# NVIDIA-AI-IOT/redtail

Hardware: AMD Instinct MI355X
Metric: stereo pairs/sec, ResNet18-2D 1257x369 (higher is better)
Workload: dtype f32

## Files before the change

include/rt_stereo.h:

```cpp
#ifndef RT_STEREO_H
#define RT_STEREO_H

#include <stddef.h>
#include <stdint.h>

#ifdef __cplusplus
extern "C" {
#endif

typedef void* rtStream;

enum { RT_F32 = 0, RT_F16 = 1 };
enum { RT_NCHW = 0, RT_NC2HW2 = 1 };
enum { RT_ACT_NONE = 0, RT_ACT_ELU = 1, RT_ACT_SIGMOID = 2 };
enum { RT_E_BADARG = -1, RT_E_UNSUPPORTED = -2, RT_E_NODEVICE = -3, RT_E_NOMEM = -4, RT_E_RUNTIME = -5 };

const char* rt_last_error_string(void);
const char* rt_backend_name(void);
int rt_device_count(void);
int rt_set_device(int ordinal);

int rt_malloc(void** dptr, size_t bytes);
int rt_free(void* dptr);
int rt_memcpy_h2d(void* dst, const void* src, size_t bytes, rtStream stream);
// ... 67 lines not shown
int rt_preprocess_frames_u8_lr(const void* left_u8, const void* right_u8, int src_h, int src_w, int64_t src_step, int encoding,
                               void* left_dst, void* right_dst, int dst_h, int dst_w, int batch, rtStream stream);
enum { RT_DISP_NET = 0, RT_DISP_PIXELS_F32 = 1, RT_DISP_KITTI_U16 = 2 };
int rt_lr_consistency(const void* net_disp, int batch, int H, int W, float scale, float max_diff_px, void* out, int out_kind,
                      void* mask_u8, void* right_out, void* valid_count, rtStream stream);

size_t rt_speckle_workspace_bytes(int batch, int H, int W);
int rt_disparity_speckle(const void* disp_px, const void* mask_u8, int batch, int H, int W, int max_size, float max_diff_px,
                         void* out, void* out_mask_u8, void* valid_count, void* workspace, size_t workspace_bytes, rtStream stream);

int rt_preprocess_frames_u8_cv(const void* left_u8, const void* right_u8, int src_h, int src_w, int64_t src_step, int encoding,
                               void* left_dst, void* right_dst, int dst_h, int dst_w, int batch, int mirror_twin, rtStream stream);
int rt_disparity_to_frame(const void* disp_px, const void* mask_u8, int batch, int H, int W, void* out, int out_kind, int out_h,
                          int out_w, void* out_mask_u8, void* valid_count, rtStream stream);

typedef struct rtStereoCamera {
    float fx, fy, cx, cy;
    float baseline;
    float doffs;
} rtStereoCamera;
enum { RT_DEPTH_M_F32 = 0, RT_DEPTH_MM_U16 = 1 };
size_t rt_points_workspace_bytes(int batch, int out_h, int out_w);
int rt_disparity_to_points(const void* disp_px, const void* mask_u8, int batch, int H, int W, int out_h, int out_w,
                           const rtStereoCamera* cam, float min_depth, float max_depth, const void* color_u8, int64_t color_step,
                           int encoding, void* disp_out, int disp_kind, void* out_mask_u8, void* valid_count, void* depth, int depth_kind,
                           void* points, void* points_compact, void* count, void* workspace, size_t workspace_bytes, rtStream stream);

typedef struct rtVoxelGrid { float origin[3]; float leaf[3]; int dims[3]; } rtVoxelGrid;
size_t rt_voxel_workspace_bytes(int batch, int capacity, const rtVoxelGrid* grid);
int rt_points_voxel_grid(const void* points, const void* count, int batch, int capacity, const rtVoxelGrid* grid, int min_points,
                         void* voxels, int out_capacity, void* out_count, void* out_cell_u32, void* out_n_u32,
                         void* workspace, size_t workspace_bytes, rtStream stream);

typedef struct rtRectifyCamera {
    double fx, fy, cx, cy;
    double d[8];
    double iR[9];
} rtRectifyCamera;
int rt_rectify_camera_from_info(const double K[9], const double* D, int n_d, const double R[9], const double P[12], rtRectifyCamera* out);
int rt_rectify_frames_u8(const void* left_u8, const void* right_u8, int src_h, int src_w, int64_t src_step, int encoding,
                         const rtRectifyCamera* cam_left, const rtRectifyCamera* cam_right,
                         void* left_dst, void* right_dst, int dst_h, int dst_w, int64_t dst_step, int batch, rtStream stream);
int rt_rectify_maps(const rtRectifyCamera* cam, int dst_h, int dst_w, void* map_x_f32, void* map_y_f32, rtStream stream);
int rt_remap_frames_u8(const void* left_u8, const void* right_u8, int src_h, int src_w, int64_t src_step, int encoding,
                       const void* map_x_left, const void* map_y_left, const void* map_x_right, const void* map_y_right,
                       void* left_dst, void* right_dst, int dst_h, int dst_w, int64_t dst_step, int batch, rtStream stream);

enum { RT_WIRE_MONO8 = 16, RT_WIRE_MONO16 = 17,
       RT_WIRE_BAYER_RGGB8 = 18, RT_WIRE_BAYER_BGGR8 = 19, RT_WIRE_BAYER_GBRG8 = 20, RT_WIRE_BAYER_GRBG8 = 21,
       RT_WIRE_YUV422 = 22 , RT_WIRE_YUV422_YUY2 = 23  };
int rt_decode_frames_u8(const void* left_wire, const void* right_wire, int h, int w, int64_t wire_step, int wire_encoding,
                        void* left_u8, void* right_u8, int64_t dst_step, int dst_encoding , int batch, rtStream stream);

int rt_disparity_to_color(const void* disp_px, int batch, int H, int W, float max_disp, void* dst_rgb8, int64_t dst_step, rtStream stream);
int rt_viz_mosaic_u8(const void* left_u8, const void* right_u8, int src_h, int src_w, int64_t src_step, int encoding,
                     const void* disp_px, int H, int W, float max_disp, void* dst_rgb8, int64_t dst_step, int batch, rtStream stream);

typedef struct rtConvPlan rtConvPlan;

typedef struct rtConv2dDesc {
    int Cin, Cout;
    int Hin, Win;
    int KH, KW;
    int stride;
    int pad_h, pad_w;
    int act;
    int has_residual;
    int dtype;
    int flags;
} rtConv2dDesc;

#define RT_CONV_EXACT_FP32 1

int rt_conv2d_plan_create(rtConvPlan** plan, const rtConv2dDesc* desc, const void* weights_host,
                          const void* bias_host);
int rt_deconv2d_plan_create(rtConvPlan** plan, const rtConv2dDesc* desc, const void* weights_host,
                            const void* bias_host);

int rt_resblock_plan_create(rtConvPlan** plan, const rtConv2dDesc* d1, const void* w1, const void* b1,
                            const rtConv2dDesc* d2, const void* w2, const void* b2);

int rt_resblock_plan_supports_split(const rtConvPlan* plan);
int rt_resblock_plan_set_split(rtConvPlan* plan, int x_split, int y_split);

int rt_conv_plan_set_pitch(rtConvPlan* plan, int in_pitch, int out_pitch);
int rt_conv_plan_set_batch_strides(rtConvPlan* plan, int64_t x_bstride, int64_t y_bstride, int64_t r_bstride);

int rt_conv_plan_set_io_types(rtConvPlan* plan, int x_dtype, int y_dtype);

int rt_conv_plan_supports_il8(const rtConvPlan* plan);
int rt_conv_plan_set_layouts(rtConvPlan* plan, int x_il8, int y_il8, int r_il8);

int rt_conv_plan_set_softarg(rtConvPlan* plan, int mode);

typedef struct rtConv3dDesc {
    int C, K;
    int D, H, W;
    int kernel[3];
    int stride[3];
    int pad_start[3];
    int pad_end[3];
    int act;
    int out_dchw;
    int has_residual;
    int dtype;
    int out_depth;
    int in_pad_end;
    int cv_fold;
    int flags;
} rtConv3dDesc;

int rt_conv3d_plan_create(rtConvPlan** plan, const rtConv3dDesc* desc, const void* weights_host,
                          const void* bias_host);
int rt_conv3d_transpose_plan_create(rtConvPlan** plan, const rtConv3dDesc* desc, const int in_dims[3],
                                    const void* weights_host, const void* bias_host);

int rt_has_experimental(void);

int rt_conv_plan_input_limit(const rtConvPlan* plan, float* limit);
int rt_check_range(const void* x, int64_t rows, int64_t valid, int64_t pitch, int dtype, float limit, float* max_abs, int64_t* violations,
                   rtStream stream);

int rt_hash_buffer(const void* x, size_t bytes, unsigned long long* out_dev, rtStream stream);

int rt_conv_plan_out_dims(const rtConvPlan* plan, int dims[4]);
int rt_conv_enqueue(const rtConvPlan* plan, const void* x, void* y, const void* residual, int batch,
                    rtStream stream);
#define RT_HINT_THROUGHPUT 1
int rt_conv_enqueue_hint(const rtConvPlan* plan, const void* x, void* y, const void* residual, int batch,
                         rtStream stream, int hints);
int rt_conv_plan_supports_twin_input(const rtConvPlan* plan);
int rt_conv_enqueue_twin_input(const rtConvPlan* plan, const void* x, const void* x2, void* y, int batch, rtStream stream, int hints);

size_t rt_conv_plan_workspace_bytes(const rtConvPlan* plan, int batch);
int rt_conv_enqueue_ws(const rtConvPlan* plan, const void* x, void* y, const void* residual, int batch, void* workspace,
                       size_t workspace_bytes, rtStream stream, int hints);
int rt_conv_plan_destroy(rtConvPlan* plan);

typedef struct rtComm rtComm;
#define RT_COMM_ID_BYTES 128
int rt_comm_unique_id(void* id_bytes);
int rt_comm_init_rank(rtComm** comm, int world, int rank, const void* id_bytes);
int rt_comm_init_all(rtComm** comms, int ndev, const int* devices);
int rt_comm_adopt(rtComm** comm, void* nccl_comm);
int rt_comm_info(const rtComm* comm, int* world, int* rank);
int rt_comm_broadcast(rtComm* comm, void* host_buf, size_t bytes, int root, rtStream stream);
int rt_comm_group_start(void);
int rt_comm_group_end(void);
int rt_comm_destroy(rtComm* comm);

#ifdef __cplusplus
}
#endif
#endif
```

redtail_amd/capi.py:

```python
import ctypes
import os
from ctypes import POINTER, c_char_p, c_double, c_float, c_int, c_int64, c_size_t, c_void_p

ROOT = os.path.dirname(os.path.dirname(os.path.abspath(__file__)))
_LIB_DIR = os.environ.get("RT_LIB_DIR") or os.path.join(ROOT, "redtail_amd", "lib")
HIP_LIB = os.path.join(_LIB_DIR, "librt_stereo_hip.so")
HOST_LIB = os.path.join(_LIB_DIR, "libnvstereo_inference.so")

RT_F32, RT_F16 = 0, 1
RT_NCHW, RT_NC2HW2 = 0, 1
RT_ACT_NONE, RT_ACT_ELU, RT_ACT_SIGMOID = 0, 1, 2


RT_ENC_BGR8, RT_ENC_RGB8, RT_ENC_BGRA8, RT_ENC_RGBA8 = 0, 1, 2, 3
ENC_BYTES = {RT_ENC_BGR8: 3, RT_ENC_RGB8: 3, RT_ENC_BGRA8: 4, RT_ENC_RGBA8: 4}
RT_WIRE_MONO8, RT_WIRE_MONO16 = 16, 17
RT_WIRE_BAYER_RGGB8, RT_WIRE_BAYER_BGGR8, RT_WIRE_BAYER_GBRG8, RT_WIRE_BAYER_GRBG8 = 18, 19, 20, 21
RT_WIRE_YUV422, RT_WIRE_YUV422_YUY2 = 22, 23
WIRE_BYTES = {RT_WIRE_MONO8: 1, RT_WIRE_MONO16: 2, RT_WIRE_BAYER_RGGB8: 1, RT_WIRE_BAYER_BGGR8: 1, RT_WIRE_BAYER_GBRG8: 1, RT_WIRE_BAYER_GRBG8: 1,
              RT_WIRE_YUV422: 2, RT_WIRE_YUV422_YUY2: 2}
RT_DISP_NET, RT_DISP_PIXELS_F32, RT_DISP_KITTI_U16 = 0, 1, 2
RT_DEPTH_M_F32, RT_DEPTH_MM_U16 = 0, 1
RT_HINT_THROUGHPUT = 1
RT_CONV_EXACT_FP32 = 1
# ... 62 lines not shown
    "rt_stream_sync": (c_int, [c_void_p]),
    "rt_stream_wait_event": (c_int, [c_void_p, c_void_p]),
    "rt_event_create": (c_int, [POINTER(c_void_p)]),
    "rt_event_create_ordering": (c_int, [POINTER(c_void_p)]),
    "rt_event_destroy": (c_int, [c_void_p]),
    "rt_event_record": (c_int, [c_void_p, c_void_p]),
    "rt_event_elapsed_ms": (c_int, [c_void_p, c_void_p, POINTER(c_float)]),
    "rt_elu": (c_int, [c_void_p, c_void_p, c_int64, c_int, c_void_p]),
    "rt_add_act": (c_int, [c_void_p, c_void_p, c_void_p, c_int64, c_int, c_int, c_void_p]),
    "rt_activation": (c_int, [c_void_p, c_void_p, c_int64, c_int, c_int, c_void_p]),
    "rt_corr_cost_volume": (c_int, [c_void_p, c_void_p, c_void_p] + [c_int] * 7 + [c_void_p]),
    "rt_corr_cost_volume_flags": (c_int, [c_void_p, c_void_p, c_void_p] + [c_int] * 7 + [ctypes.c_uint, c_void_p]),
    "rt_cost_volume": (c_int, [c_void_p, c_void_p, c_void_p] + [c_int] * 6 + [c_void_p]),
    "rt_softargmax": (c_int, [c_void_p, c_void_p] + [c_int] * 6 + [c_void_p]),
    "rt_corr_softargmax": (c_int, [c_void_p, c_void_p, c_void_p] + [c_int] * 6 + [c_int64, c_int, c_void_p]),
    "rt_corr_softargmax_flags": (c_int, [c_void_p, c_void_p, c_void_p] + [c_int] * 6 + [c_int64, c_int, ctypes.c_uint, c_void_p]),
    "rt_corr_softargmax_pitched": (c_int, [c_void_p, c_void_p, c_void_p] + [c_int] * 8 + [c_int64, c_int, c_void_p]),
    "rt_corr_softargmax_il": (c_int, [c_void_p, c_void_p, c_void_p] + [c_int] * 8 + [c_int64, c_void_p]),
    "rt_corr_softargmax_il_slot": (c_int, [c_void_p, c_void_p, c_void_p] + [c_int] * 8 + [c_int64, c_int, c_void_p]),
    "rt_corr_softargmax_il8_f16": (c_int, [c_void_p, c_void_p, c_void_p] + [c_int] * 8 + [c_int64, c_int, c_void_p]),
    "rt_permute4d": (c_int, [c_void_p, c_void_p] + [c_int] * 5 + [POINTER(c_int), c_int, c_void_p]),
    "rt_convert_format": (c_int, [c_void_p, c_void_p, c_int, c_int, c_int64, c_int, c_int, c_void_p]),
    "rt_pad_d": (c_int, [c_void_p, c_void_p, c_int, c_int, c_int64, c_int, c_int, c_void_p]),
    "rt_slice_d": (c_int, [c_void_p, c_void_p, c_int, c_int, c_int64, c_int, c_int, c_int, c_void_p]),
    "rt_concat_channels": (c_int, [c_void_p, c_void_p, c_int, c_int, c_int, c_int, c_int64, c_int, c_void_p]),
    "rt_conv2d_plan_create": (c_int, [POINTER(c_void_p), POINTER(Conv2dDesc), c_void_p, c_void_p]),
    "rt_deconv2d_plan_create": (c_int, [POINTER(c_void_p), POINTER(Conv2dDesc), c_void_p, c_void_p]),
    "rt_resblock_plan_create": (c_int, [POINTER(c_void_p), POINTER(Conv2dDesc), c_void_p, c_void_p, POINTER(Conv2dDesc), c_void_p,
                                        c_void_p]),
    "rt_conv3d_plan_create": (c_int, [POINTER(c_void_p), POINTER(Conv3dDesc), c_void_p, c_void_p]),
    "rt_conv3d_transpose_plan_create": (c_int, [POINTER(c_void_p), POINTER(Conv3dDesc), POINTER(c_int), c_void_p,
                                                c_void_p]),
    "rt_preprocess_bgr8": (c_int, [c_void_p, c_int, c_int, c_void_p, c_int, c_int, c_int, c_void_p]),
    "rt_disparity_to_u16": (c_int, [c_void_p, c_void_p, c_int64, ctypes.c_float, c_void_p]),
    "rt_preprocess_frames_u8": (c_int, [c_void_p, c_void_p, c_int, c_int, c_int64, c_int, c_void_p, c_void_p, c_int, c_int, c_int,
                                        c_void_p]),
    "rt_disparity_scale": (c_int, [c_void_p, c_void_p, c_int64, ctypes.c_float, c_void_p]),
    "rt_preprocess_frames_u8_lr": (c_int, [c_void_p, c_void_p, c_int, c_int, c_int64, c_int, c_void_p, c_void_p, c_int, c_int, c_int,
                                           c_void_p]),
    "rt_lr_consistency": (c_int, [c_void_p, c_int, c_int, c_int, c_float, c_float, c_void_p, c_int, c_void_p, c_void_p, c_void_p, c_void_p]),
    "rt_preprocess_frames_u8_cv": (c_int, [c_void_p, c_void_p, c_int, c_int, c_int64, c_int, c_void_p, c_void_p, c_int, c_int, c_int, c_int,
                                           c_void_p]),
    "rt_disparity_to_frame": (c_int, [c_void_p, c_void_p, c_int, c_int, c_int, c_void_p, c_int, c_int, c_int, c_void_p, c_void_p, c_void_p]),
    "rt_points_workspace_bytes": (c_size_t, [c_int, c_int, c_int]),
    "rt_disparity_to_points": (c_int, [c_void_p, c_void_p, c_int, c_int, c_int, c_int, c_int, POINTER(StereoCamera), c_float, c_float, c_void_p,
                                       c_int64, c_int, c_void_p, c_int, c_void_p, c_void_p, c_void_p, c_int, c_void_p, c_void_p, c_void_p,
                                       c_void_p, c_size_t, c_void_p]),
    "rt_speckle_workspace_bytes": (c_size_t, [c_int, c_int, c_int]),
    "rt_voxel_workspace_bytes": (c_size_t, [c_int, c_int, c_void_p]),
    "rt_points_voxel_grid": (c_int, [c_void_p, c_void_p, c_int, c_int, c_void_p, c_int, c_void_p, c_int, c_void_p, c_void_p, c_void_p, c_void_p,
                                     c_size_t, c_void_p]),
    "rt_disparity_speckle": (c_int, [c_void_p, c_void_p, c_int, c_int, c_int, c_int, c_float, c_void_p, c_void_p, c_void_p, c_void_p, c_size_t,
                                     c_void_p]),
    "rt_rectify_camera_from_info": (c_int, [POINTER(c_double), POINTER(c_double), c_int, POINTER(c_double), POINTER(c_double),
                                            POINTER(RectifyCamera)]),
    "rt_rectify_frames_u8": (c_int, [c_void_p, c_void_p, c_int, c_int, c_int64, c_int, POINTER(RectifyCamera), POINTER(RectifyCamera), c_void_p,
                                     c_void_p, c_int, c_int, c_int64, c_int, c_void_p]),
    "rt_rectify_maps": (c_int, [POINTER(RectifyCamera), c_int, c_int, c_void_p, c_void_p, c_void_p]),
    "rt_remap_frames_u8": (c_int, [c_void_p, c_void_p, c_int, c_int, c_int64, c_int, c_void_p, c_void_p, c_void_p, c_void_p, c_void_p, c_void_p,
                                   c_int, c_int, c_int64, c_int, c_void_p]),
    "rt_decode_frames_u8": (c_int, [c_void_p, c_void_p, c_int, c_int, c_int64, c_int, c_void_p, c_void_p, c_int64, c_int, c_int, c_void_p]),
    "rt_disparity_to_color": (c_int, [c_void_p, c_int, c_int, c_int, c_float, c_void_p, c_int64, c_void_p]),
    "rt_viz_mosaic_u8": (c_int, [c_void_p, c_void_p, c_int, c_int, c_int64, c_int, c_void_p, c_int, c_int, c_float, c_void_p, c_int64, c_int,
                                 c_void_p]),
    "rt_conv_plan_input_limit": (c_int, [c_void_p, POINTER(c_float)]),
    "rt_has_experimental": (c_int, []),
    "rt_graph_begin_capture": (c_int, [c_void_p]),
    "rt_graph_end_capture": (c_int, [c_void_p, POINTER(c_void_p)]),
    "rt_graph_launch": (c_int, [c_void_p, c_void_p]),
    "rt_graph_destroy": (c_int, [c_void_p]),
    "rt_check_range": (c_int, [c_void_p, c_int64, c_int64, c_int64, c_int, c_float, POINTER(c_float), POINTER(c_int64), c_void_p]),
    "rt_hash_buffer": (c_int, [c_void_p, c_size_t, c_void_p, c_void_p]),
    "rt_conv_plan_out_dims": (c_int, [c_void_p, POINTER(c_int)]),
    "rt_conv_plan_set_pitch": (c_int, [c_void_p, c_int, c_int]),
    "rt_conv_plan_set_batch_strides": (c_int, [c_void_p, c_int64, c_int64, c_int64]),
    "rt_conv_plan_set_io_types": (c_int, [c_void_p, c_int, c_int]),
    "rt_conv_plan_supports_il8": (c_int, [c_void_p]),
    "rt_conv_plan_set_layouts": (c_int, [c_void_p, c_int, c_int, c_int]),
    "rt_conv_plan_set_softarg": (c_int, [c_void_p, c_int]),
    "rt_conv_plan_supports_twin_input": (c_int, [c_void_p]),
    "rt_conv_enqueue_twin_input": (c_int, [c_void_p, c_void_p, c_void_p, c_void_p, c_int, c_void_p, c_int]),
    "rt_resblock_plan_supports_split": (c_int, [c_void_p]),
    "rt_resblock_plan_set_split": (c_int, [c_void_p, c_int, c_int]),
    "rt_conv_enqueue": (c_int, [c_void_p, c_void_p, c_void_p, c_void_p, c_int, c_void_p]),
    "rt_conv_enqueue_hint": (c_int, [c_void_p, c_void_p, c_void_p, c_void_p, c_int, c_void_p, c_int]),
    "rt_conv_plan_workspace_bytes": (ctypes.c_size_t, [c_void_p, c_int]),
    "rt_conv_enqueue_ws": (c_int, [c_void_p, c_void_p, c_void_p, c_void_p, c_int, c_void_p, ctypes.c_size_t, c_void_p, c_int]),
    "rt_conv_plan_destroy": (c_int, [c_void_p]),
    "rt_comm_unique_id": (c_int, [c_void_p]),
    "rt_comm_init_rank": (c_int, [POINTER(c_void_p), c_int, c_int, c_void_p]),
    "rt_comm_init_all": (c_int, [POINTER(c_void_p), c_int, POINTER(c_int)]),
    "rt_comm_adopt": (c_int, [POINTER(c_void_p), c_void_p]),
    "rt_comm_info": (c_int, [c_void_p, POINTER(c_int), POINTER(c_int)]),
    "rt_comm_broadcast": (c_int, [c_void_p, c_void_p, c_size_t, c_int, c_void_p]),
    "rt_comm_group_start": (c_int, []),
    "rt_comm_group_end": (c_int, []),
    "rt_comm_destroy": (c_int, [c_void_p]),
}
RT_COMM_ID_BYTES = 128


def _ptr(x):
    if x is None:
        return None
    if isinstance(x, int):
        return x
    if hasattr(x, "data_ptr"):
        return x.data_ptr()
    if hasattr(x, "ctypes"):
        return x.ctypes.data
    raise TypeError("cannot take the address of %r" % type(x))


def _host_weights(a, dtype, what):
    if a is not None and hasattr(a, "dtype") and hasattr(a, "ctypes"):
        want = "float16" if dtype == RT_F16 else "float32"
        if a.dtype.name != want:
            raise TypeError("%s: expected a %s array, got %s" % (what, want, a.dtype))
        if not a.flags["C_CONTIGUOUS"]:
            raise TypeError("%s: array is not C-contiguous" % what)
    return a


class KernelLib:

    def __init__(self, path=None):
        emulated = path is not None
        path = path or HIP_LIB
        if not os.path.exists(path):
            raise RtError("native library %s is missing -- run `python -m redtail_amd.build` "
                          "(there is no Python fallback for the HIP path)" % path)
        self.path = path
        self.lib = ctypes.CDLL(path, mode=ctypes.RTLD_GLOBAL)
        for name, (res, args) in KERNEL_SYMBOLS.items():
            fn = getattr(self.lib, name)
            fn.restype, fn.argtypes = res, args
        if not emulated and self.lib.rt_device_count() < 1:
            raise RtError("no HIP device visible: the Stereo DNN path runs on MI355X only")

    def check(self, rc, what=""):
        if rc != 0:
            raise RtError("%s failed (%d): %s" % (what, rc, self.lib.rt_last_error_string().decode()))

    def backend(self):
        return self.lib.rt_backend_name().decode()

    def elu(self, x, y, n, dtype=RT_F32, stream=None):
        self.check(self.lib.rt_elu(_ptr(x), _ptr(y), n, dtype, stream), "rt_elu")

    def add_act(self, a, b, y, n, act, dtype=RT_F32, stream=None):
        self.check(self.lib.rt_add_act(_ptr(a), _ptr(b), _ptr(y), n, act, dtype, stream), "rt_add_act")

    def activation(self, x, y, n, act, dtype=RT_F32, stream=None):
        self.check(self.lib.rt_activation(_ptr(x), _ptr(y), n, act, dtype, stream), "rt_activation")

    def corr_cost_volume(self, l, r, cv, batch, C, H, W, D, dtype=RT_F32, fmt=RT_NCHW, stream=None, flags=0):
        self.check(self.lib.rt_corr_cost_volume_flags(_ptr(l), _ptr(r), _ptr(cv), batch, C, H, W, D, dtype, fmt, flags, stream)
                   if flags else self.lib.rt_corr_cost_volume(_ptr(l), _ptr(r), _ptr(cv), batch, C, H, W, D, dtype, fmt, stream),
                   "rt_corr_cost_volume")

    def preprocess_bgr8(self, src, src_h, src_w, dst, dst_h, dst_w, batch=1, stream=None):
        self.check(self.lib.rt_preprocess_bgr8(_ptr(src), src_h, src_w, _ptr(dst), dst_h, dst_w, batch, stream),
                   "rt_preprocess_bgr8")

    def disparity_to_u16(self, disp, out, n, scale, stream=None):
        self.check(self.lib.rt_disparity_to_u16(_ptr(disp), _ptr(out), n, scale, stream), "rt_disparity_to_u16")

    def preprocess_frames_u8(self, left, right, src_h, src_w, src_step, encoding, left_dst, right_dst, dst_h, dst_w, batch=1,
                             stream=None):
        self.check(self.lib.rt_preprocess_frames_u8(_ptr(left), _ptr(right), src_h, src_w, src_step, encoding, _ptr(left_dst),
                                                    _ptr(right_dst), dst_h, dst_w, batch, stream), "rt_preprocess_frames_u8")

    def disparity_scale(self, disp, out, n, scale, stream=None):
        self.check(self.lib.rt_disparity_scale(_ptr(disp), _ptr(out), n, scale, stream), "rt_disparity_scale")

    def preprocess_frames_u8_lr(self, left, right, src_h, src_w, src_step, encoding, left_dst, right_dst, dst_h, dst_w, batch=1,
                                stream=None):
        self.check(self.lib.rt_preprocess_frames_u8_lr(_ptr(left), _ptr(right), src_h, src_w, src_step, encoding, _ptr(left_dst),
                                                       _ptr(right_dst), dst_h, dst_w, batch, stream), "rt_preprocess_frames_u8_lr")

    def lr_consistency(self, net_disp, batch, h, w, scale, max_diff_px, out, kind=1, mask=None, right_out=None, valid_count=None,
                       stream=None):
        self.check(self.lib.rt_lr_consistency(_ptr(net_disp), batch, h, w, scale, max_diff_px, _ptr(out), kind, _ptr(mask),
                                              _ptr(right_out), _ptr(valid_count), stream), "rt_lr_consistency")

    def preprocess_frames_u8_cv(self, left, right, src_h, src_w, src_step, encoding, left_dst, right_dst, dst_h, dst_w, batch=1,
                                mirror_twin=False, stream=None):
        self.check(self.lib.rt_preprocess_frames_u8_cv(_ptr(left), _ptr(right), src_h, src_w, src_step, encoding, _ptr(left_dst),
                                                       _ptr(right_dst), dst_h, dst_w, batch, int(bool(mirror_twin)), stream),
                   "rt_preprocess_frames_u8_cv")

    def disparity_to_frame(self, disp_px, batch, h, w, out, out_h, out_w, kind=1, mask=None, out_mask=None, valid_count=None, stream=None):
        self.check(self.lib.rt_disparity_to_frame(_ptr(disp_px), _ptr(mask), batch, h, w, _ptr(out), kind, out_h, out_w, _ptr(out_mask),
                                                  _ptr(valid_count), stream), "rt_disparity_to_frame")

    def rectify_frames_u8(self, left, right, src_h, src_w, src_step, encoding, cam_left, cam_right, left_dst, right_dst, dst_h, dst_w,
                          dst_step, batch=1, stream=None):
        self.check(self.lib.rt_rectify_frames_u8(_ptr(left), _ptr(right), src_h, src_w, src_step, encoding,
                                                 ctypes.byref(cam_left) if cam_left is not None else None,
                                                 ctypes.byref(cam_right) if cam_right is not None else None, _ptr(left_dst), _ptr(right_dst),
                                                 dst_h, dst_w, dst_step, batch, stream), "rt_rectify_frames_u8")

    def rectify_maps(self, cam, dst_h, dst_w, map_x, map_y, stream=None):
        self.check(self.lib.rt_rectify_maps(ctypes.byref(cam) if cam is not None else None, dst_h, dst_w, _ptr(map_x), _ptr(map_y), stream),
                   "rt_rectify_maps")

    def remap_frames_u8(self, left, right, src_h, src_w, src_step, encoding, map_x_left, map_y_left, map_x_right, map_y_right, left_dst,
                        right_dst, dst_h, dst_w, dst_step, batch=1, stream=None):
        self.check(self.lib.rt_remap_frames_u8(_ptr(left), _ptr(right), src_h, src_w, src_step, encoding, _ptr(map_x_left), _ptr(map_y_left),
                                               _ptr(map_x_right), _ptr(map_y_right), _ptr(left_dst), _ptr(right_dst), dst_h, dst_w, dst_step,
                                               batch, stream), "rt_remap_frames_u8")

    def decode_frames_u8(self, left_wire, right_wire, h, w, wire_step, wire_encoding, left_dst, right_dst, dst_step, dst_encoding=RT_ENC_BGR8,
                         batch=1, stream=None):
        self.check(self.lib.rt_decode_frames_u8(_ptr(left_wire), _ptr(right_wire), h, w, wire_step, wire_encoding, _ptr(left_dst), _ptr(right_dst),
                                                dst_step, dst_encoding, batch, stream), "rt_decode_frames_u8")

# ... 100 lines not shown

    def hash_buffer(self, x, bytes, stream=None):
        out, value = c_void_p(), ctypes.c_uint64()
        self.check(self.lib.rt_malloc(ctypes.byref(out), 8), "rt_malloc")
        try:
            self.check(self.lib.rt_hash_buffer(_ptr(x), bytes, out, stream), "rt_hash_buffer")
            self.check(self.lib.rt_memcpy_d2h(ctypes.byref(value), out, 8, stream), "rt_memcpy_d2h")
            self.check(self.lib.rt_stream_sync(stream), "rt_stream_sync")
        finally:
            self.lib.rt_free(out)
        return value.value

    def conv2d_plan(self, w_host, b_host, Cin, Cout, Hin, Win, k, stride, pad, act=0, has_residual=False,
                    dtype=RT_F32, transposed=False, flags=0):
        d = Conv2dDesc(Cin, Cout, Hin, Win, k, k, stride, pad, pad, act, int(has_residual), dtype, flags)
        _host_weights(w_host, dtype, "conv2d_plan weights"); _host_weights(b_host, dtype, "conv2d_plan bias")
        plan = c_void_p()
        fn = self.lib.rt_deconv2d_plan_create if transposed else self.lib.rt_conv2d_plan_create
        self.check(fn(ctypes.byref(plan), ctypes.byref(d), _ptr(w_host), _ptr(b_host)), "conv2d plan")
        return ConvPlan(self, plan)

    def resblock_plan(self, w1, b1, w2, b2, C, Cmid, H, W, act1=RT_ACT_ELU, act2=RT_ACT_ELU, dtype=RT_F32):
        d1 = Conv2dDesc(C, Cmid, H, W, 3, 3, 1, 1, 1, act1, 0, dtype)
        d2 = Conv2dDesc(Cmid, C, H, W, 3, 3, 1, 1, 1, act2, 1, dtype)
        plan = c_void_p()
        self.check(self.lib.rt_resblock_plan_create(ctypes.byref(plan), ctypes.byref(d1), _ptr(w1), _ptr(b1), ctypes.byref(d2),
                                                    _ptr(w2), _ptr(b2)), "resblock plan")
        return ConvPlan(self, plan)

    def conv3d_plan(self, w_host, b_host, C, K, dims, kernel, stride, pad_start, pad_end, act=0, out_dchw=False,
                    has_residual=False, dtype=RT_F32, transposed_in_dims=None, out_depth=0, in_pad_end=0, cv_fold=0):
        d = Conv3dDesc(C, K, dims[0], dims[1], dims[2], (c_int * 3)(*kernel), (c_int * 3)(*stride),
                       (c_int * 3)(*pad_start), (c_int * 3)(*pad_end), act, int(out_dchw), int(has_residual), dtype,
                       out_depth, in_pad_end, cv_fold)
        plan = c_void_p()
        if transposed_in_dims is None:
            rc = self.lib.rt_conv3d_plan_create(ctypes.byref(plan), ctypes.byref(d), _ptr(w_host), _ptr(b_host))
        else:
            ind = (c_int * 3)(*transposed_in_dims)
            rc = self.lib.rt_conv3d_transpose_plan_create(ctypes.byref(plan), ctypes.byref(d), ind, _ptr(w_host),
                                                          _ptr(b_host))
        self.check(rc, "conv3d plan")
        return ConvPlan(self, plan)


class ConvPlan:
    def __init__(self, klib, handle):
        self.klib, self.handle = klib, handle
        dims = (c_int * 4)()
        klib.check(klib.lib.rt_conv_plan_out_dims(handle, dims), "rt_conv_plan_out_dims")
        self.out_dims = tuple(dims)

    def set_pitch(self, in_pitch, out_pitch):
        self.klib.check(self.klib.lib.rt_conv_plan_set_pitch(self.handle, in_pitch, out_pitch), "rt_conv_plan_set_pitch")

    def set_batch_strides(self, x_bstride, y_bstride, r_bstride=0):
        self.klib.check(self.klib.lib.rt_conv_plan_set_batch_strides(self.handle, x_bstride, y_bstride, r_bstride), "rt_conv_plan_set_batch_strides")

    def set_io_types(self, x_dtype, y_dtype):
        self.klib.check(self.klib.lib.rt_conv_plan_set_io_types(self.handle, x_dtype, y_dtype), "rt_conv_plan_set_io_types")

    def input_limit(self):
        v = c_float()
        self.klib.check(self.klib.lib.rt_conv_plan_input_limit(self.handle, ctypes.byref(v)), "rt_conv_plan_input_limit")
        return v.value

    def supports_il8(self):
        return bool(self.klib.lib.rt_conv_plan_supports_il8(self.handle))

    def il_caps(self):
        return int(self.klib.lib.rt_conv_plan_supports_il8(self.handle))

    def set_layouts(self, x_il8, y_il8, r_il8=False):
        self.klib.check(self.klib.lib.rt_conv_plan_set_layouts(self.handle, int(x_il8), int(y_il8), int(r_il8)), "rt_conv_plan_set_layouts")

    def enqueue_twin_input(self, x, x2, y, batch=1, stream=None, hints=0):
        self.klib.check(self.klib.lib.rt_conv_enqueue_twin_input(self.handle, _ptr(x), _ptr(x2), _ptr(y), batch, stream, hints), "rt_conv_enqueue_twin_input")

    def supports_split(self):
        return bool(self.klib.lib.rt_resblock_plan_supports_split(self.handle))

    def set_split(self, x_split, y_split):
        self.klib.check(self.klib.lib.rt_resblock_plan_set_split(self.handle, int(x_split), int(y_split)), "rt_resblock_plan_set_split")

    def set_softarg(self, mode):
        self.klib.check(self.klib.lib.rt_conv_plan_set_softarg(self.handle, int(mode)), "rt_conv_plan_set_softarg")

    def enqueue(self, x, y, residual=None, batch=1, stream=None, hints=0):
        self.klib.check(self.klib.lib.rt_conv_enqueue_hint(self.handle, _ptr(x), _ptr(y), _ptr(residual), batch, stream, hints),
                        "rt_conv_enqueue")

    def destroy(self):
        if self.handle:
            self.klib.lib.rt_conv_plan_destroy(self.handle)
            self.handle = None

    def __del__(self):
        try:
            self.destroy()
        except Exception:
            pass


RT_MODEL_RESNET18_2D, RT_MODEL_NVSMALL, RT_MODEL_NVTINY, RT_MODEL_RESNET18 = 0, 1, 2, 3
RT_RESIZE_AREA_DOWN, RT_RESIZE_CV_AREA = 0, 1
RT_GEOM_NET, RT_GEOM_FRAME = 0, 1
MODEL_IDS = {"resnet18_2D": RT_MODEL_RESNET18_2D, "nvsmall": RT_MODEL_NVSMALL, "nvtiny": RT_MODEL_NVTINY,
             "resnet18": RT_MODEL_RESNET18}

NET_SYMBOLS = {
    "rt_net_create": (c_int, [POINTER(c_void_p), c_int, c_int, c_int, c_int, c_int, c_int, c_char_p]),
    "rt_net_create_from_memory": (c_int, [POINTER(c_void_p), c_int, c_int, c_int, c_int, c_int, c_int, c_void_p,
                                          c_size_t]),
    "rt_net_serialize": (c_int, [c_void_p, c_void_p, c_size_t, POINTER(c_size_t)]),
    "rt_net_create_from_plan": (c_int, [POINTER(c_void_p), c_void_p, c_size_t]),
    "rt_net_execute": (c_int, [c_void_p, c_void_p, c_void_p, c_void_p, c_int, c_void_p]),
    "rt_net_execute_frames": (c_int, [c_void_p, c_void_p, c_void_p, c_int, c_int, c_int64, c_int, c_void_p, c_int, c_int, c_void_p]),
    "rt_net_execute_frames_lr": (c_int, [c_void_p, c_void_p, c_void_p, c_int, c_int, c_int64, c_int, c_void_p, c_int, c_void_p, c_void_p,
                                         c_void_p, c_float, c_int, c_void_p]),
    "rt_net_execute_frames_viz": (c_int, [c_void_p, c_void_p, c_void_p, c_int, c_int, c_int64, c_int, c_void_p, c_void_p, c_int64, c_float,
                                          c_float, c_void_p, c_void_p, c_int, c_void_p]),
    "rt_net_execute_frames_ex": (c_int, [c_void_p, c_void_p, c_void_p]),
    "rt_net_execute_frames_3d": (c_int, [c_void_p, c_void_p, c_void_p, c_void_p]),
    "rt_net_execute_frames_raw": (c_int, [c_void_p, c_void_p, c_void_p, c_void_p, c_void_p]),
    "rt_net_execute_frames_filtered": (c_int, [c_void_p, c_void_p, c_void_p, c_void_p, c_void_p, c_void_p]),
    "rt_net_execute_frames_camera": (c_int, [c_void_p, c_void_p, c_void_p, c_void_p, c_void_p, c_void_p, c_void_p]),
    "rt_net_execute_frames_voxels": (c_int, [c_void_p, c_void_p, c_void_p, c_void_p, c_void_p, c_void_p, c_void_p, c_void_p]),
    "rt_net_profile": (c_int, [c_void_p, c_void_p, c_void_p, c_void_p, c_int, c_char_p, c_size_t]),
    "rt_net_num_layers": (c_int, [c_void_p]),
    "rt_net_num_launches": (c_int, [c_void_p]),
    "rt_net_set_streams": (c_int, [c_void_p, c_int]),
    "rt_net_set_graph": (c_int, [c_void_p, c_int]),
    "rt_net_create_broadcast": (c_int, [POINTER(c_void_p), c_int, c_int, c_int, c_int, c_int, c_int, c_void_p, c_size_t, c_void_p, c_int]),
    "rt_net_weights_crc32": (c_int, [c_void_p, POINTER(ctypes.c_uint32)]),
    "rt_net_weights_image": (c_int, [c_void_p, POINTER(c_void_p), POINTER(c_size_t)]),
    "rt_net_create_opt": (c_int, [POINTER(c_void_p), c_void_p]),
    "rt_net_set_debug": (c_int, [c_void_p, c_int]),
    "rt_net_set_launch_trace": (c_int, [c_void_p, c_int]),
    "rt_net_read_launch_trace": (c_int, [c_void_p, POINTER(ctypes.c_ulonglong), c_int]),
    "rt_net_launch_name": (c_char_p, [c_void_p, c_int]),
    "rt_net_read_launch_output": (ctypes.c_longlong, [c_void_p, c_int, c_void_p, ctypes.c_longlong]),
    "rt_net_destroy": (c_int, [c_void_p]),
    "rt_net_last_error": (c_char_p, []),
}


class NetOptions(ctypes.Structure):
    _fields_ = [("model", c_int), ("width", c_int), ("height", c_int), ("max_batch", c_int), ("weights_dtype", c_int), ("max_disp", c_int),
                ("weights_path", c_char_p), ("blob", c_void_p), ("bytes", c_size_t), ("flags", ctypes.c_uint), ("comm", c_void_p), ("root", c_int)]


class FrameCall(ctypes.Structure):
    _fields_ = [("struct_bytes", c_size_t), ("left_u8", c_void_p), ("right_u8", c_void_p), ("src_h", c_int), ("src_w", c_int),
                ("src_step", c_int64), ("encoding", c_int), ("resize", c_int), ("disp", c_void_p), ("disp_kind", c_int), ("geometry", c_int),
                ("max_diff_px", c_float), ("mask_u8", c_void_p), ("valid_count", c_void_p), ("batch", c_int)]


class DepthCall(ctypes.Structure):
    _fields_ = [("struct_bytes", c_size_t), ("camera", StereoCamera), ("min_depth", c_float), ("max_depth", c_float), ("depth", c_void_p),
                ("depth_kind", c_int), ("points", c_void_p), ("points_compact", c_void_p), ("count", c_void_p)]


class RectifyCall(ctypes.Structure):
    _fields_ = [("struct_bytes", c_size_t), ("left", RectifyCamera), ("right", RectifyCamera), ("left_rect_u8", c_void_p),
                ("right_rect_u8", c_void_p), ("rect_step", c_int64)]

# ... 418 lines not shown
```

redtail_amd/csrc/host/engine.cpp:

```cpp
#include <algorithm>
#include <cassert>
#include <cstdlib>
#include <cstdio>
#include <cstring>
#include <cstdint>
#include <map>
#include <set>
#include <memory>
#include <sstream>
#include <string>
#include <vector>

#include "NvInfer.h"
#include "plugin_internal.h"
#include "rt_stereo.h"

namespace nvinfer1 {
namespace {

const char* knob(const char* name) {
    static const bool on = [] { const char* e = std::getenv("RT_DEV_KNOBS"); return e && std::atoi(e) != 0; }();
    return on ? std::getenv(name) : nullptr;
}

// ... 351 lines not shown
    std::string blob;
    void* data() const override { return const_cast<char*>(blob.data()); }
    std::size_t size() const override { return blob.size(); }
    DataType type() const override { return DataType::kINT8; }
    void destroy() override { delete this; }
};

class EngineImpl : public ICudaEngine {
public:
    EngineImpl(NetworkImpl& net, int max_batch, bool half2, ILogger& log, bool exact_fp32 = false);
    ~EngineImpl() override;
    bool ok() const { return ok_; }

    int getNbBindings() const override { return (int)bindings_.size(); }
    int getBindingIndex(const char* name) const override {
        for (size_t i = 0; i < bindings_.size(); i++)
            if (tensors_[bindings_[i]]->name == name) return (int)i;
        return -1;
    }
    const char* getBindingName(int i) const override { return tensors_[bindings_[i]]->name.c_str(); }
    bool bindingIsInput(int i) const override { return tensors_[bindings_[i]]->is_input; }
    Dims getBindingDimensions(int i) const override { return tensors_[bindings_[i]]->dims; }
    DataType getBindingDataType(int) const override { return DataType::kFLOAT; }
    int getMaxBatchSize() const override { return max_batch_; }
    int getNbLayers() const override { return (int)ops_.size(); }
    std::size_t getWorkspaceSize() const override { return 2 * workspace_bytes_; }
    IHostMemory* serialize() const override;
    IExecutionContext* createExecutionContext() override {
        for (auto& l : layers_)
            if (l->plugin && l->plugin->initialize() != 0)
                log_.log(ILogger::Severity::kERROR, (l->name + ": plugin initialize() failed").c_str());
        return new ContextImpl(*this);
    }
    void destroy() override { delete this; }

    std::vector<std::unique_ptr<TensorImpl>> tensors_;
    std::vector<std::unique_ptr<LayerData>> layers_;
    std::vector<int> bindings_;
    std::vector<Op> ops_;
    int max_batch_;
    size_t workspace_bytes_ = 0;
    bool two_streams_ = false;
    std::vector<size_t> issue_sync_;
    ILogger& log_;

    static int64_t sampleElems(const TensorImpl& t) {
        if (t.dims.nbDims != 3) return (int64_t)volume(t.dims);
        return (int64_t)(t.cpad ? t.cpad : t.dims.d[0]) * t.dims.d[1] * (t.pitch ? t.pitch : t.dims.d[2]);
    }

private:
    int root(int t) const {
        while (tensors_[t]->alias_of >= 0) t = tensors_[t]->alias_of;
        return t;
    }
    bool concatFoldable(size_t ci) const;
    void applySampleStrides();
    int consumers(int t) const {
        int n = 0;
        for (auto& l : layers_)
            for (auto* i : l->in)
                if (i->id == t) n++;
        return n + (tensors_[t]->is_output ? 1 : 0);
    }
    LayerData* soleConsumer(int t) const {
        if (consumers(t) != 1 || tensors_[t]->is_output) return nullptr;
        for (auto& l : layers_)
            for (auto* i : l->in)
                if (i->id == t) return l.get();
        return nullptr;
    }
    static IStereoPlugin* stereo(LayerData* l) { return l && l->plugin ? dynamic_cast<IStereoPlugin*>(l->plugin) : nullptr; }
    static bool isKind(LayerData* l, Kind k) { auto* s = stereo(l); return s && s->kind() == k; }
    bool lower();
    void assignStreams();
    void planIssueOrder();
    void assignPitch();
    void foldConcats();
    void foldCostVolumes();
    void assignHalf3D();
    void assignInterleaved3D();
    void fuseSoftargmax3D();
    void fuseResBlocks();
    void mergeSiamese();
    bool ok_ = false;
    bool half2_ = false;
    bool exact_fp32_ = false;
    std::vector<IPlugin*> half_plugins_;
    std::vector<int> half_kinds_;
public:
    std::vector<std::unique_ptr<char[]>> weight_store_;
};

EngineImpl::EngineImpl(NetworkImpl& net, int max_batch, bool half2, ILogger& log, bool exact_fp32)
    : max_batch_(max_batch), log_(log), half2_(half2), exact_fp32_(exact_fp32 || (knob("RT_CONV_EXACT_FP32") && atoi(knob("RT_CONV_EXACT_FP32")) != 0)) {
    tensors_ = std::move(net.tensors_);
    layers_ = std::move(net.layers_);
    for (auto* t : net.inputs_) bindings_.push_back(t->id);
    for (auto* t : net.outputs_) bindings_.push_back(t->id);
    net.inputs_.clear();
    net.outputs_.clear();
    net.ilayers_.clear();

    for (auto& l : layers_) {
        if (!l->plugin) continue;
        std::vector<Dims> in_dims, out_dims;
        for (auto* t : l->in) in_dims.push_back(t->dims);
        for (auto* t : l->out) out_dims.push_back(t->dims);
        if (l->plugin_ext) {
            auto* ext = static_cast<IPluginExt*>(l->plugin);
            DataType type = ext->supportsFormat(DataType::kFLOAT, PluginFormat::kNCHW) ? DataType::kFLOAT : DataType::kHALF;
            PluginFormat fmt = PluginFormat::kNCHW;
            if (!ext->supportsFormat(type, fmt)) fmt = PluginFormat::kNC2HW2;
            if (type != DataType::kFLOAT) { half_plugins_.push_back(l->plugin); half_kinds_.push_back(fmt == PluginFormat::kNCHW ? 1 : 2); }
            ext->configureWithFormat(in_dims.data(), (int)in_dims.size(), out_dims.data(), (int)out_dims.size(), type, fmt, max_batch_);
        } else {
            l->plugin->configure(in_dims.data(), (int)in_dims.size(), out_dims.data(), (int)out_dims.size(), max_batch_);
        }
        workspace_bytes_ = std::max(workspace_bytes_, l->plugin->getWorkspaceSize(max_batch_));
    }
    ok_ = lower();
    if (ok_)
        for (auto& op : ops_) {
            if (op.kind != OpKind::kPlugin) continue;
            auto it = std::find(half_plugins_.begin(), half_plugins_.end(), op.plugin);
            if (it != half_plugins_.end()) op.half_kind = half_kinds_[it - half_plugins_.begin()];
        }
    if (ok_) assignStreams();
    if (ok_) assignPitch();
    if (ok_) fuseResBlocks();
    if (ok_) assignStreams();
    if (ok_) foldConcats();
    if (ok_) foldCostVolumes();
    if (ok_) assignHalf3D();
    if (ok_) assignInterleaved3D();
    if (ok_) fuseSoftargmax3D();
    if (ok_) mergeSiamese();
    if (ok_) applySampleStrides();
    if (ok_) assignStreams();
    if (ok_) planIssueOrder();
    if (ok_)
        for (auto& op : ops_)
            if (op.kind == OpKind::kConv3D && op.plugin) workspace_bytes_ = std::max(workspace_bytes_, op.plugin->getWorkspaceSize(max_batch_));
    workspace_bytes_ = (workspace_bytes_ + 255) / 256 * 256;
}

EngineImpl::~EngineImpl() {
    for (auto& op : ops_)
        if (op.plan) rt_conv_plan_destroy(op.plan);
    for (auto& l : layers_)
        if (l->plugin) l->plugin->terminate();
}

static bool isIdentityScale(const LayerData& l) {
    auto val = [](const Weights& w, float dflt) {
        if (w.count == 0 || !w.values) return dflt;
        if (w.type == DataType::kHALF) {
            uint16_t h;
            std::memcpy(&h, w.values, 2);
            return h == 0 ? 0.f : (h == 0x3c00 ? 1.f : -1234.f);
        }
        float f;
        std::memcpy(&f, w.values, 4);
        return f;
    };
    return l.scale_mode == ScaleMode::kUNIFORM && val(l.shift, 0.f) == 0.f && val(l.scale, 1.f) == 1.f && val(l.power, 1.f) == 1.f;
}

bool EngineImpl::lower() {
    std::vector<bool> done(layers_.size(), false);
    auto index_of = [&](LayerData* l) {
        for (size_t i = 0; i < layers_.size(); i++)
            if (layers_[i].get() == l) return (int)i;
        return -1;
    };
    auto fail = [&](const std::string& msg) {
        log_.log(ILogger::Severity::kERROR, msg.c_str());
        return false;
    };
    const bool fuse = knob("RT_NO_FUSION") == nullptr;

    for (size_t li = 0; li < layers_.size(); li++) {
        if (done[li]) continue;
        LayerData* l = layers_[li].get();
        done[li] = true;
        Op op;
        op.name = l->name;
        op.lays.push_back((int)li);
        for (auto* t : l->in) op.in.push_back(t->id);
        op.out = l->out[0]->id;

        switch (l->type) {
            case LayerType::kSCALE: {
                if (!isIdentityScale(*l)) return fail(l->name + ": only identity scale layers occur in the Stereo DNN graphs");
                l->out[0]->alias_of = l->in[0]->id;
                continue;
            }
            case LayerType::kSHUFFLE: {
                l->out[0]->alias_of = l->in[0]->id;
                continue;
            }
            case LayerType::kCONVOLUTION:
            case LayerType::kDECONVOLUTION: {
                const bool deconv = l->type == LayerType::kDECONVOLUTION;
                const Dims& x = l->in[0]->dims;
                if (l->ksize.h() != l->ksize.w() || l->stride.h() != l->stride.w())
                    return fail(l->name + ": non-square kernels / strides are not used by the Stereo DNN graphs");
                TensorImpl* cur = l->out[0];
                int resid = -1, act = RT_ACT_NONE;
                if (fuse) {
                    LayerData* nx = soleConsumer(cur->id);
                    if (nx && nx->type == LayerType::kELEMENTWISE && nx->ew == ElementWiseOperation::kSUM) {
                        TensorImpl* other = nx->in[0] == cur ? nx->in[1] : nx->in[0];
                        auto same_dims = [](const Dims& a, const Dims& b) {
                            if (a.nbDims != b.nbDims) return false;
                            for (int i = 0; i < a.nbDims; i++)
                                if (a.d[i] != b.d[i]) return false;
                            return true;
                        };
// ... 381 lines not shown
        size_t h[2] = {0, 0};
        int turn = 1;
        while (issue_sync_.size() < ops_.size()) {
            int st = turn;
            if (h[st] >= q[st].size() || !ready(ops_[q[st][h[st]]])) st ^= 1;
            if (h[st] >= q[st].size() || !ready(ops_[q[st][h[st]]])) break;
            const size_t i = q[st][h[st]++];
            issue_sync_.push_back(i);
            for (int r = ops_[i].out; r >= 0; r = tensors_[r]->alias_of) produced[r] = 1;
            for (int r = ops_[i].twin_out; r >= 0; r = tensors_[r]->alias_of) produced[r] = 1;
            turn = st ^ 1;
        }
        if (issue_sync_.size() != ops_.size()) issue_sync_.clear();
    }
}

void EngineImpl::fuseResBlocks() {
    const char* e = knob("RT_RB");
    const bool force = e && atoi(e) != 0;
    const bool h2 = half2_ && !knob("RT_NO_F16");
    if ((e && !force) || knob("RT_NO_FUSION") || knob("RT_NO_RB") || knob("RT_NO_S3") || exact_fp32_ || (h2 && (knob("RT_NO_RBH") || knob("RT_NO_F16MMA")))) return;
    int fused = 0;
    for (size_t ia = 0; ia < ops_.size(); ia++) {
        Op& a = ops_[ia];
        if (a.kind != OpKind::kConv || !a.conv_layer || a.conv_layer->type != LayerType::kCONVOLUTION || a.resid >= 0) continue;
        if (tensors_[a.out]->is_output) continue;
        int ib = -1, uses = 0;
        for (size_t j = 0; j < ops_.size(); j++) {
            if (j == ia) continue;
            for (int x : ops_[j].in)
                if (root(x) == root(a.out)) { uses++; ib = (int)j; }
            if (ops_[j].resid >= 0 && root(ops_[j].resid) == root(a.out)) uses += 2;
        }
        if (uses != 1 || ib < (int)ia) continue;
        Op& b = ops_[ib];
        if (b.kind != OpKind::kConv || !b.conv_layer || b.conv_layer->type != LayerType::kCONVOLUTION || b.in.size() != 1 ||
            root(b.in[0]) != root(a.out) || b.resid < 0 || root(b.resid) != root(a.in[0]))
            continue;
        auto desc = [&](const Op& op, bool resid) {
            const LayerData* l = op.conv_layer;
            const Dims& x = l->in[0]->dims;
            rtConv2dDesc d{};
            d.Cin = x.d[0]; d.Cout = l->nb_maps; d.Hin = x.d[1]; d.Win = x.d[2];
            d.KH = l->ksize.h(); d.KW = l->ksize.w(); d.stride = l->stride.h();
            d.pad_h = l->padding.h(); d.pad_w = l->padding.w();
            d.act = op.act; d.has_residual = resid;
            d.dtype = l->kernel.type == DataType::kHALF ? RT_F16 : RT_F32;
            return d;
        };
        const rtConv2dDesc d1 = desc(a, false), d2 = desc(b, true);
        const TensorImpl &x = *tensors_[root(a.in[0])], &y = *tensors_[root(b.out)];
        {
            bool ok = d1.Cin == 32 && d1.Cout == 32 && d2.Cout == 32 && a.act == RT_ACT_ELU && b.act == RT_ACT_ELU;
            ok = ok && x.il8 && y.il8 && x.f16 == h2 && y.f16 == h2;
            if (h2 && !ok) continue;
            if (force ? (!ok && !rt_has_experimental()) : !(ok && ((d1.Win + 29) / 30) * ((d1.Hin + 15) / 16) >= 200)) continue;
        }
        const LayerData *la = a.conv_layer, *lb = b.conv_layer;
        rtConvPlan* rb = nullptr;
        if (rt_resblock_plan_create(&rb, &d1, la->kernel.values, la->bias.count ? la->bias.values : nullptr, &d2, lb->kernel.values,
                                    lb->bias.count ? lb->bias.values : nullptr) != 0)
            continue;
        bool cfg = (!(x.pitch || y.pitch) || rt_conv_plan_set_pitch(rb, x.pitch, y.pitch) == 0) &&
                   rt_conv_plan_set_io_types(rb, x.f16 ? RT_F16 : RT_F32, y.f16 ? RT_F16 : RT_F32) == 0 &&
                   (!(x.il8 || y.il8) || rt_conv_plan_set_layouts(rb, x.il8, y.il8, x.il8) == 0);
        if (!cfg) {
            rt_conv_plan_destroy(rb);
            continue;
        }
        rt_conv_plan_destroy(a.plan);
        rt_conv_plan_destroy(b.plan);
        a.plan = rb;
        a.out = b.out;
        a.resid = b.resid;
        a.act = b.act;
        a.name += "+" + b.name;
        a.lays.insert(a.lays.end(), b.lays.begin(), b.lays.end());
        ops_.erase(ops_.begin() + ib);
        fused++;
    }
    if (fused)
        log_.log(ILogger::Severity::kINFO, ("engine: " + std::to_string(fused) + " residual blocks fused into one launch each; " +
                                            std::to_string(ops_.size()) + " launches").c_str());
    if (!fused || knob("RT_NO_RBD")) return;
    auto tower = [&](const Op& op) { return op.kind == OpKind::kConv && op.plan && rt_resblock_plan_supports_split(op.plan) != 0; };
    int nsplit = 0;
    for (size_t ia = 0; ia < ops_.size(); ia++) {
        const Op& a = ops_[ia];
        if (!tower(a) || root(a.out) != a.out) continue;
        TensorImpl& t = *tensors_[a.out];
        if (t.is_output || t.is_input || t.bstride != 0 || t.cpad != 0 || !t.il8 || t.f16) continue;
        int readers = 0;
        bool ok = true;
        for (size_t j = 0; j < ops_.size(); j++) {
            const Op& b = ops_[j];
            bool reads = b.resid >= 0 && root(b.resid) == t.id;
            for (int x : b.in) reads = reads || root(x) == t.id;
            if (!reads) continue;
            readers++;
            ok = ok && j > ia && tower(b) && b.in.size() == 1 && root(b.in[0]) == t.id && b.resid >= 0 && root(b.resid) == t.id;
        }
        if (readers == 1 && ok) { t.split = true; nsplit++; }
    }
    if (!nsplit) return;
    for (Op& op : ops_) {
        if (!tower(op)) continue;
        const bool xs = tensors_[root(op.in[0])]->split, ys = tensors_[root(op.out)]->split;
        if ((xs || ys) && rt_resblock_plan_set_split(op.plan, xs, ys) != 0) {
            log_.log(ILogger::Severity::kERROR, rt_last_error_string());
            ok_ = false;
            return;
        }
    }
    log_.log(ILogger::Severity::kINFO, ("engine: " + std::to_string(nsplit) + " tensors between tower blocks stored pre-split (fp16 hi / lo operand pairs)").c_str());
}

void EngineImpl::mergeSiamese() {
    if (knob("RT_NO_SIAMESE") || knob("RT_NO_FUSION")) return;
    std::vector<int> ins;
    for (int b : bindings_)
        if (tensors_[b]->is_input) ins.push_back(b);
    if (ins.size() != 2) return;
    auto same_dims = [](const Dims& a, const Dims& b) {
        if (a.nbDims != b.nbDims) return false;
        for (int i = 0; i < a.nbDims; i++)
            if (a.d[i] != b.d[i]) return false;
        return true;
    };
    if (!same_dims(tensors_[ins[0]]->dims, tensors_[ins[1]]->dims)) return;
    auto same_weights = [](const Weights& a, const Weights& b) {
        if (a.count != b.count || a.type != b.type) return false;
        if (a.count == 0) return true;
        const size_t es = a.type == DataType::kHALF ? 2 : 4;
        return a.values && b.values && (a.values == b.values || std::memcmp(a.values, b.values, (size_t)a.count * es) == 0);
    };
    std::vector<int> twin_t(tensors_.size(), -1), twin_l(layers_.size(), -1);
    std::vector<char> is_right(layers_.size(), 0);
    twin_t[ins[0]] = ins[1];
    auto same_layer = [&](const LayerData& a, const LayerData& b) {
        if (a.type != b.type || a.in.size() != b.in.size() || a.out.size() != b.out.size()) return false;
        for (size_t i = 0; i < a.in.size(); i++)
            if (twin_t[a.in[i]->id] != b.in[i]->id) return false;
        for (size_t i = 0; i < a.out.size(); i++)
            if (!same_dims(a.out[i]->dims, b.out[i]->dims)) return false;
        switch (a.type) {
            case LayerType::kCONVOLUTION:
            case LayerType::kDECONVOLUTION:
                return a.nb_maps == b.nb_maps && a.ksize.h() == b.ksize.h() && a.ksize.w() == b.ksize.w() && a.stride.h() == b.stride.h() &&
                       a.stride.w() == b.stride.w() && a.padding.h() == b.padding.h() && a.padding.w() == b.padding.w() &&
                       same_weights(a.kernel, b.kernel) && same_weights(a.bias, b.bias);
            case LayerType::kSCALE: return isIdentityScale(a) && isIdentityScale(b);
            case LayerType::kELEMENTWISE: return a.ew == b.ew;
            case LayerType::kACTIVATION: return a.act == b.act;
            case LayerType::kPLUGIN: {
                IStereoPlugin *pa = a.plugin ? dynamic_cast<IStereoPlugin*>(a.plugin) : nullptr, *pb = b.plugin ? dynamic_cast<IStereoPlugin*>(b.plugin) : nullptr;
                return pa && pb && pa->kind() == Kind::kElu && pb->kind() == Kind::kElu;
            }
            default: return false;
        }
    };
    for (size_t ia = 0; ia < layers_.size(); ia++) {
        const LayerData& a = *layers_[ia];
        if (is_right[ia] || a.in.empty()) continue;
        bool have = true;
        for (auto* t : a.in) have = have && twin_t[t->id] >= 0;
        if (!have) continue;
        for (size_t ib = 0; ib < layers_.size(); ib++) {
            if (ib == ia || is_right[ib] || twin_l[ib] >= 0 || !same_layer(a, *layers_[ib])) continue;
            twin_l[ia] = (int)ib;
            is_right[ib] = 1;
            for (size_t i = 0; i < a.out.size(); i++) twin_t[a.out[i]->id] = layers_[ib]->out[i]->id;
            break;
        }
    }
    auto plain = [&](const TensorImpl& t) { return !t.is_input && !t.is_output && t.alias_of < 0 && t.bstride == 0 && t.twin_of < 0 && !t.has_twin; };
    auto pairable = [&](int l, int r) {
        if (l < 0 || r < 0 || l == r) return false;
        const TensorImpl &a = *tensors_[l], &b = *tensors_[r];
        return plain(a) && plain(b) && same_dims(a.dims, b.dims) && a.pitch == b.pitch && a.f16 == b.f16 && a.il8 == b.il8 && a.split == b.split && b.cpad == 0;
    };
    int merged = 0;
    for (size_t ia = 0; ia < ops_.size(); ia++) {
        Op& a = ops_[ia];
        if (a.kind != OpKind::kConv || a.twin || a.in.size() != 1 || a.lays.empty() || twin_l[a.lays[0]] < 0) continue;
        int ib = -1;
        for (size_t j = 0; j < ops_.size() && ib < 0; j++) {
            const Op& b = ops_[j];
            if (j == ia || b.kind != OpKind::kConv || b.twin || b.lays.size() != a.lays.size() || b.in.size() != 1 || b.act != a.act) continue;
            bool eq = true;
            for (size_t k = 0; k < a.lays.size(); k++) eq = eq && twin_l[a.lays[k]] == b.lays[k];
            if (eq) ib = (int)j;
        }
        if (ib < 0) continue;
        const Op& b = ops_[ib];
        const bool from_bindings = root(a.in[0]) == ins[0] && root(b.in[0]) == ins[1] && a.resid < 0 && !knob("RT_NO_TWIN_INPUT") &&
                                   tensors_[a.in[0]]->alias_off == 0 && tensors_[b.in[0]]->alias_off == 0 && rt_conv_plan_supports_twin_input(a.plan) != 0;
        if ((!from_bindings && (root(a.in[0]) != a.in[0] || root(b.in[0]) != b.in[0])) || root(a.out) != a.out || root(b.out) != b.out) continue;
// ... 1150 lines not shown
```

redtail_amd/csrc/kernels/conv_mfma.hip.h:

```cpp
#pragma once
#include <type_traits>
#include "common.hip.h"

namespace rt {

struct ZSlice {
    int pad_y, pad_x;
    int Ho, Wo;
    int ch_row;
    unsigned tap_mask;
    int64_t y_off;
    int64_t w_off;
    int64_t r_off;
    int64_t r_off_il8;
    int64_t y_off_il8;
    int64_t r_off_il4;
};

struct ConvArgs {
    const float* x;
    float* y;
    const float* w;
    const float* bias;
    const float* resid;
    unsigned long long* dbg;
    const float* zeros;
    const ZSlice* zs;
    const int* ch_off;
    int CinPad;
    int Cout;
    int Hi, Wi;
    int x_pitch;
    int Ho, Wo;
    int pad_y, pad_x;
    int nz;
    int tiles_x;
    int act;
    int xcd_order;
    int64_t x_bstride;
    int64_t y_bstride;
    int64_t y_cstride;
    int64_t y_zstride;
    int64_t y_off;
    int y_ystride, y_xstride;
    int64_t r_cstride;
    int64_t r_bstride;
    int r_il8;
    int batch;
    int cin_real;
    int64_t x_cstride;
    const int* ch_shift;
    int w_exact;
    int z_inner;
    int nb_inner;
    int dw_seg, dw_nseg, dw_cpc, dw_ntiles;
    const float* x2;
    int x2_from;
};

#define RT_WG_TILE_NB(p, tile, zi, n, nblk)                                                         \
    int tile = blockIdx.x;                                                                          \
    if ((p).xcd_order) {                           \
        const int nwg_ = gridDim.x, q_ = nwg_ >> 3, r_ = nwg_ & 7;                                  \
        const int xcd_ = blockIdx.x & 7, idx_ = blockIdx.x >> 3;                                    \
        tile = (xcd_ < r_ ? xcd_ * (q_ + 1) : r_ * (q_ + 1) + (xcd_ - r_) * q_) + idx_;             \
    }                                                                                               \
    int nblk = blockIdx.y;                                                                          \
    if ((p).nb_inner > 0) { nblk = tile % (p).nb_inner; tile /= (p).nb_inner; }                     \
    int zi, n;                                                                                      \
    if ((p).z_inner) { zi = tile % (p).nz; tile /= (p).nz; n = blockIdx.z; }                        \
    else { zi = blockIdx.z % (p).nz; n = blockIdx.z / (p).nz; }
#define RT_WG_TILE(p, tile, zi, n) RT_WG_TILE_NB(p, tile, zi, n, nblk_unused_); (void)nblk_unused_;

#ifdef RT_KERNEL_TIMING
#define RT_TSTAMP() do { if (dbgp && tid == 0 && dbi < 16) dbgp[dbi++] = __builtin_amdgcn_s_memtime(); } while (0)
#else
#define RT_TSTAMP() do { } while (0)
#endif

#ifndef RT_ABLATE
#define RT_ABLATE 0
#endif
constexpr bool kAblGather = (RT_ABLATE & 1) != 0;
constexpr bool kAblWLoad = (RT_ABLATE & 2) != 0;
constexpr bool kAblLdsWr = (RT_ABLATE & 4) != 0;
constexpr bool kAblBarrier = (RT_ABLATE & 8) != 0;
constexpr bool kAblResid = (RT_ABLATE & 16) != 0;
constexpr bool kAblStore = (RT_ABLATE & 32) != 0;
constexpr bool kAblLdsRd = (RT_ABLATE & 64) != 0;
constexpr bool kAblXform = (RT_ABLATE & 128) != 0;
constexpr bool kAblMfma = (RT_ABLATE & 256) != 0;
__device__ __forceinline__ void wg_barrier() { if (!kAblBarrier) __syncthreads(); }

template <int N> struct VecOf;
template <> struct VecOf<2> { typedef float type __attribute__((ext_vector_type(2))); };
template <> struct VecOf<4> { typedef float type __attribute__((ext_vector_type(4))); };

template <int KH, int KW, int S, int TY, int TXW, int NBW, int CC, int NW = 4, bool WLDS = true>
struct ConvCfg {
    static constexpr int TX = 32 * TXW;
    static constexpr int NB = 32 * NBW;
    static constexpr int TAPS = KH * KW;
    static constexpr int CPG = CC / 2;
    static constexpr int PR = (TY - 1) * S + KH;
    static constexpr int PC = (TX - 1) * S + KW;
    static constexpr int NPIX = PR * PC;
    static constexpr int IN_ELEMS = CC * NPIX;
    static constexpr int W_ELEMS = TAPS * CC * NB;
    static constexpr int NPAR = NW == 1 ? 2 : 1;
    static constexpr int NPART = NW == 1 ? 1 : NW / 2;
    static constexpr int NKP = ((NPIX + NPART - 1) / NPART + 63) / 64;
    static constexpr int NTHR = 64 * NW;
    static constexpr int NK_W = (W_ELEMS / 4 + NTHR - 1) / NTHR;
    static constexpr int WT = TY * TXW / NW;
    static constexpr int NBUF = 1;
    static constexpr int MINW = (WT * NBW == 1 && NW == 4 && TY == 4) ? 5 : (WT * NBW == 1 && NW == 8 ? 4 : 1);
    static_assert(NW == 1 || NW == 2 || NW == 4 || NW == 8, "1, 2, 4 or 8 waves per workgroup");
    static_assert((TY * TXW) % NW == 0, "tile must split evenly over the waves");
    static_assert(WLDS || true, "");
    static_assert(CC == 4 || CC == 8, "CC/2 k-steps are fetched by one ds_read_b64 / ds_read_b128");
    static_assert(W_ELEMS % 4 == 0, "weight slab is copied as float4");
};

template <int KH, int KW, int S, int TY, int TXW, int NBW, int CC, int NW, bool WLDS, typename TIN = float, typename TOUT = float, bool YIL = false>
__global__ void __launch_bounds__(64 * NW, (ConvCfg<KH, KW, S, TY, TXW, NBW, CC, NW, WLDS>::MINW))
conv_mfma_f32_kernel(ConvArgs p) {
    static_assert(!YIL || std::is_same<TOUT, float>::value, "interleaved output: fp32");
    constexpr unsigned ESX = Io<TIN>::ES, ESY = Io<TOUT>::ES;
    using Cfg = ConvCfg<KH, KW, S, TY, TXW, NBW, CC, NW, WLDS>;
    constexpr int TX = Cfg::TX, NB = Cfg::NB, PC = Cfg::PC, WT = Cfg::WT, CPG = Cfg::CPG;
    constexpr int NPIX = Cfg::NPIX, NKP = Cfg::NKP, TAPS = Cfg::TAPS, NPAR = Cfg::NPAR, NTHR = Cfg::NTHR;
    typedef typename VecOf<CPG>::type vec_t;

    constexpr int NBUF = Cfg::NBUF;
    __shared__ __attribute__((aligned(16))) float sIn[NBUF][Cfg::IN_ELEMS];
    __shared__ __attribute__((aligned(16))) float sW[NBUF][WLDS ? Cfg::W_ELEMS : 4];

    const int tid = threadIdx.x;
    const int lane = tid & 63;
    const int half = lane >> 5, l31 = lane & 31;
// ... 349 lines not shown
```

redtail_amd/csrc/kernels/conv_split.hip.h:

```cpp
#pragma once
#include <type_traits>
#include "common.hip.h"
#include "conv_mfma.hip.h"

namespace rt {

constexpr float kSplitScale = 2048.f;
constexpr float kSplitInv = 1.f / 2048.f;

struct S3Split {
    f16x4 hi, lo;
};
__device__ static __forceinline__ S3Split s3_split(f32x4 v) {
    S3Split s;
#ifdef HIPEMU
#pragma unroll
    for (int j = 0; j < 4; j++) {
        const _Float16 h = (_Float16)v[j];
        s.hi[j] = h;
        s.lo[j] = (_Float16)((v[j] - (float)h) * kSplitScale);
    }
#else
    unsigned h[2], l[2];
#pragma unroll
// ... 152 lines not shown
            for (int q = 0; q < 4; q++) rr[q] = f32x4{0.f, 0.f, 0.f, 0.f};
        }

        f32x16 acc_m, acc_c;
#pragma unroll
        for (int r = 0; r < 16; r++) { acc_m[r] = 0.f; acc_c[r] = 0.f; }
        const char* xb = sX[buf] + b_off;
#pragma unroll
        for (int t = 0; t < 9; t++) {
            const int r = t / 3, s = t % 3;
#pragma unroll
            for (int c = 0; c < 2; c++) {
                const char* bp = xb + (r * PC + s) * PXB + c * 32;
                const f16x8 bh = *reinterpret_cast<const f16x8*>(bp);
                const f16x8 bl = *reinterpret_cast<const f16x8*>(bp + 64);
                const f16x8 ah = __builtin_bit_cast(f16x8, sW[a_off + ((t * 2 + c) * 2 + 0) * 64]);
                const f16x8 al = __builtin_bit_cast(f16x8, sW[a_off + ((t * 2 + c) * 2 + 1) * 64]);
                acc_m = __builtin_amdgcn_mfma_f32_32x32x16_f16(ah, bh, acc_m, 0, 0, 0);
                acc_c = __builtin_amdgcn_mfma_f32_32x32x16_f16(al, bh, acc_c, 0, 0, 0);
                acc_c = __builtin_amdgcn_mfma_f32_32x32x16_f16(ah, bl, acc_c, 0, 0, 0);
            }
        }

        RT_TSTAMP();
        const buf_rsrc rs_y = make_buf(elem_ptr(p.y, (int64_t)n * p.y_bstride + p.y_off, 4));
        auto epilogue = [&](auto ACT) {
#pragma unroll
            for (int q = 0; q < 4; q++) {
                f32x4 o;
#pragma unroll
                for (int e = 0; e < 4; e++)
                    o[e] = apply_act_fast(fmaf(acc_c[4 * q + e], kSplitInv, acc_m[4 * q + e]) + (bias4[q][e] + rr[q][e]), decltype(ACT)::value);
                if constexpr (YIL) {
                    const unsigned vo = (inb && 8 * q + 4 * kg < p.Cout) ? (unsigned)((oy * p.y_ystride + ox) * 4 + 4 * kg * cs32) * 4u : kBufOOB;
                    buf_store4(o, rs_y, vo, (unsigned)(8 * q * cs32) * 4u);
                } else {
                    const unsigned vo = inb ? (unsigned)(oy * p.y_ystride + ox * p.y_xstride + 4 * kg * cs32) * 4u : kBufOOB;
#pragma unroll
                    for (int e = 0; e < 4; e++)
                        buf_store(o[e], rs_y, (8 * q + 4 * kg + e < p.Cout) ? vo : kBufOOB, (unsigned)((8 * q + e) * cs32) * 4u);
                }
            }
        };
        if (act == 1) epilogue(std::integral_constant<int, 1>{});
        else if (act == 2) epilogue(std::integral_constant<int, 2>{});
        else epilogue(std::integral_constant<int, 0>{});
        RT_TSTAMP();
    }
#ifdef RT_KERNEL_TIMING
    __builtin_amdgcn_s_waitcnt(0);
    if (dbgp && tid == 0) { dbgp[14] = __builtin_amdgcn_s_memtime(); dbgp[15] = __builtin_amdgcn_s_memrealtime() - rt0; }
#endif
}

}

namespace rt {

template <int KH, int KW, int S, int NW_ = 4>
struct S3Cfg {
    static constexpr int NW = NW_, TY = NW_, TX = 32, CC = 16, TAPS = KH * KW, NT = 64 * NW_;
    static constexpr int PR = (TY - 1) * S + KH, PC = (TX - 1) * S + KW;
    static constexpr int PCH = (PC + 1) / 2;
    static constexpr int PCL = S == 2 ? 2 * PCH : PC;
    static constexpr int NPART = NW / 4;
    static constexpr int NPIX = PR * PC, NKP = ((NPIX + NPART - 1) / NPART + 63) / 64;
    static constexpr int PXB = 80;
    static constexpr int W_SLOTS = TAPS * 2 * 2 * 32;
    static constexpr int NK_W = (W_SLOTS + NT - 1) / NT;
    static constexpr int IN_BYTES = PR * PCL * PXB, GRP_BYTES = IN_BYTES + W_SLOTS * 16;
    static constexpr int KS_MAX = NW_ != 4 ? 1 : (S == 2 ? 2 : 4);
    static constexpr int max_groups(int want) {
        int ks = want < 1 ? 1 : (want > KS_MAX ? KS_MAX : want);
        while (ks > 1 && (ks == 3 || ks * GRP_BYTES < (ks - 1) * NW * 64 * 16 * 4)) ks--;
        return ks;
    }
    static_assert(IN_BYTES % 16 == 0, "weight image alignment");
    static_assert(S == 1 || S == 2, "stride 1 or 2");
};

#ifndef RT_S3_WAVES
#define RT_S3_WAVES(S) ((S) == 2 ? 2 : 4)
#endif
template <int KH, int KW, int S, bool XIL, bool YIL, int NW = 4, typename TIN = float, typename TOUT = float>
__global__ void __launch_bounds__(64 * NW * (S3Cfg<KH, KW, S, NW>::KS_MAX)) RT_WAVES_PER_EU(RT_S3_WAVES(S)) conv_s3_kernel(ConvArgs p) {
    using Cfg = S3Cfg<KH, KW, S, NW>;
    constexpr bool XF16 = std::is_same<TIN, _Float16>::value, YF16 = std::is_same<TOUT, _Float16>::value;
    constexpr unsigned ESX = Io<TIN>::ES, ESY = Io<TOUT>::ES;
    static_assert(!XIL || !XF16, "interleaved fp16 input: conv_f16mma_kernel");
    constexpr int TY = Cfg::TY, TX = Cfg::TX, CC = Cfg::CC, TAPS = Cfg::TAPS, PC = Cfg::PC, PCL = Cfg::PCL, PXB = Cfg::PXB;
    constexpr int NKP = Cfg::NKP, NK_W = Cfg::NK_W, NT = Cfg::NT;

    constexpr int IN_BYTES = Cfg::IN_BYTES, GRP_BYTES = Cfg::GRP_BYTES;
#ifdef HIPEMU
    HIP_DYNAMIC_SHARED(char, smem)
#else
    extern __shared__ __attribute__((aligned(16))) char smem[];
#endif

    const int tid_wg = threadIdx.x;
    const int KS = Cfg::KS_MAX == 1 ? 1 : __builtin_amdgcn_readfirstlane((int)blockDim.x / NT);
    const int kgi = Cfg::KS_MAX == 1 ? 0 : __builtin_amdgcn_readfirstlane(tid_wg / NT);
    const int tid = tid_wg - kgi * NT;
    char* const sIn = smem + kgi * GRP_BYTES;
    f32x4* const sW = reinterpret_cast<f32x4*>(smem + kgi * GRP_BYTES + IN_BYTES);
#ifdef RT_KERNEL_TIMING
    unsigned long long* dbgp = (p.dbg && kgi == 0) ? p.dbg + ((size_t)(blockIdx.z * gridDim.y + blockIdx.y) * gridDim.x + blockIdx.x) * 16 : nullptr;
    int dbi = 0;
    const unsigned long long rt0 = __builtin_amdgcn_s_memrealtime();
#endif
    RT_TSTAMP();
    const int lane = tid & 63;
    const int kg = lane >> 5, l31 = lane & 31;
    const int wv = __builtin_amdgcn_readfirstlane(tid >> 6);

    RT_WG_TILE_NB(p, tile, zi, n, nblk)
    const int tx0 = (tile % p.tiles_x) * TX;
    const int ty0 = (tile / p.tiles_x) * TY;
    const char* __restrict__ xb = elem_ptr(p.x, (int64_t)n * p.x_bstride, ESX);
    const int nchunks = p.CinPad / CC;
    int pad_y = p.pad_y, pad_x = p.pad_x, Ho = p.Ho, Wo = p.Wo, ch_row = zi;
    int64_t y_off = p.y_off + (int64_t)zi * p.y_zstride, w_off = 0, r_off = y_off, r_off_il8 = y_off;
    int64_t y_off_il4 = 4 * p.y_off + (int64_t)zi * p.y_zstride, r_off_il4 = y_off_il4;
    unsigned tap_mask = ~0u;
    if (p.zs) {
        const ZSlice z = p.zs[zi];
        pad_y = z.pad_y; pad_x = z.pad_x; Ho = z.Ho; Wo = z.Wo; ch_row = z.ch_row; y_off = z.y_off; w_off = z.w_off;
        r_off = z.r_off; r_off_il8 = z.r_off_il8;
        y_off_il4 = 4 * z.y_off;
        r_off_il4 = z.r_off_il4;
        tap_mask = z.tap_mask;
    }
    const int act = p.act;

    const int sg = wv & 3, spart = wv >> 2;
    const int* __restrict__ tab = p.ch_off + (int64_t)ch_row * p.CinPad + 4 * sg;
    unsigned voff[NKP];
    int lidx[NKP], xcol[NKP];
    const int* __restrict__ shtab = p.ch_shift ? p.ch_shift + (int64_t)ch_row * p.CinPad + 4 * sg : nullptr;
#pragma unroll
    for (int k = 0; k < NKP; k++) {
        const int pidx = spart * (NKP * 64) + lane + 64 * k;
        const int pr = pidx / PC, pc = pidx - pr * PC;
        const int iy = ty0 * S - pad_y + pr, ix = tx0 * S - pad_x + pc;
        const bool own = pidx < Cfg::NPIX && lane + 64 * k < NKP * 64;
        xcol[k] = ix;
        voff[k] = (own && iy >= 0 && iy < p.Hi && ix >= 0 && ix < p.Wi) ? (unsigned)(iy * p.x_pitch + ix) * (XIL ? 16u : ESX) : kBufOOB;
        const int col = S == 2 ? (pc & 1) * Cfg::PCH + (pc >> 1) : pc;
        lidx[k] = own ? (pr * PCL + col) * PXB + sg * 8 : -1;
    }
    const char* __restrict__ wsrc = reinterpret_cast<const char*>(p.w) + (w_off + ((int64_t)nblk * nchunks) * Cfg::W_SLOTS) * 16;
    const buf_rsrc rs_w = make_buf(wsrc);

    f32x4 rin[NKP];
    f32x4 rw[NK_W];
    auto prefetch = [&](int ch) {
        if constexpr (XIL) {
            const int off = tab[ch * CC];
            const int sh = shtab ? shtab[ch * CC] : 0;
            const buf_rsrc rs = make_buf(xb, off >= 0);
#pragma unroll
            for (int k = 0; k < NKP; k++) {
                const unsigned vo = sh == 0 ? voff[k] : ((voff[k] != kBufOOB && xcol[k] >= sh) ? voff[k] - (unsigned)sh * 16u : kBufOOB);
                rin[k] = buf_load4(rs, vo, (unsigned)off * 4u);
            }
        } else {
            const int sh = shtab ? shtab[ch * CC] : 0;
#pragma unroll
            for (int j = 0; j < 4; j++) {
                const int off = tab[ch * CC + j];
                const buf_rsrc rs = make_buf(xb, off >= 0);
#pragma unroll
                for (int k = 0; k < NKP; k++) {
                    const unsigned vo = sh == 0 ? voff[k] : ((voff[k] != kBufOOB && xcol[k] >= sh) ? voff[k] - (unsigned)sh * ESX : kBufOOB);
                    rin[k][j] = Io<TIN>::load(rs, vo, (unsigned)off * ESX);
                }
            }
        }
        const unsigned so = (unsigned)ch * (unsigned)(Cfg::W_SLOTS * 16);
#pragma unroll
        for (int k = 0; k < NK_W; k++) {
            const int idx = tid + NT * k;
            rw[k] = buf_load4(rs_w, idx < Cfg::W_SLOTS ? (unsigned)idx * 16u : kBufOOB, so);
        }
    };
    auto stage_to_lds = [&]() {
#pragma unroll
        for (int k = 0; k < NKP; k++) {
            if (lidx[k] < 0) continue;
            if constexpr (XF16) {
                f16x4 h;
#pragma unroll
                for (int j = 0; j < 4; j++) h[j] = (_Float16)rin[k][j];
                *reinterpret_cast<f16x4*>(sIn + lidx[k]) = h;
            } else {
                const S3Split s = s3_split(rin[k]);
                *reinterpret_cast<f16x4*>(sIn + lidx[k]) = s.hi;
                *reinterpret_cast<f16x4*>(sIn + lidx[k] + 32) = s.lo;
            }
        }
#pragma unroll
        for (int k = 0; k < NK_W; k++) {
            const int idx = tid + NT * k;
            if (idx < Cfg::W_SLOTS) sW[idx] = rw[k];
        }
    };

    const int64_t ybase = (int64_t)n * p.y_bstride + y_off;
    const int64_t rbase = (int64_t)n * p.r_bstride + r_off;
    const int cs32 = (int)p.y_cstride, rs32 = (int)p.r_cstride;
    const int oy = ty0 + wv, ox = tx0 + l31;
    const bool inb = oy < Ho && ox < Wo;
    const bool r_il = p.r_il8 != 0;
    const int cb = nblk * 32;
    f32x4 rr[4];
    if (p.resid != nullptr && kgi == 0) {
        const buf_rsrc rs_r = make_buf(elem_ptr(p.resid, r_il ? (int64_t)n * p.r_bstride + (YF16 ? r_off_il8 : r_off_il4) : rbase, ESY));
        if (r_il && YF16) {
            const unsigned vo = inb ? (unsigned)((oy * p.y_ystride + ox * p.y_xstride) * 8 + 4 * kg) * 2u : kBufOOB;
#pragma unroll
            for (int q = 0; q < 4; q++) {
                const u32x2_t u = __builtin_amdgcn_raw_buffer_load_b64(rs_r, (cb + 8 * q + 4 * kg < p.Cout) ? vo : kBufOOB, (unsigned)((cb + 8 * q) * rs32) * 2u, 0);
#pragma unroll
                for (int e = 0; e < 4; e++) rr[q][e] = (float)__builtin_bit_cast(_Float16, (unsigned short)(u[e >> 1] >> (16 * (e & 1))));
            }
        } else if (r_il) {
            const unsigned vo = inb ? (unsigned)((oy * p.y_ystride + ox * p.y_xstride) * 4 + 4 * kg * rs32) * 4u : kBufOOB;
#pragma unroll
            for (int q = 0; q < 4; q++) rr[q] = buf_load4(rs_r, (cb + 8 * q + 4 * kg < p.Cout) ? vo : kBufOOB, (unsigned)((cb + 8 * q) * rs32) * 4u);
        } else {
            const unsigned vo = inb ? (unsigned)(oy * p.y_ystride + ox * p.y_xstride + 4 * kg * rs32) * ESY : kBufOOB;
#pragma unroll
            for (int q = 0; q < 4; q++)
#pragma unroll
                for (int e = 0; e < 4; e++)
                    rr[q][e] = Io<TOUT>::load(rs_r, (cb + 8 * q + 4 * kg + e < p.Cout) ? vo : kBufOOB, (unsigned)((cb + 8 * q + e) * rs32) * ESY);
        }
    } else {
#pragma unroll
        for (int q = 0; q < 4; q++) rr[q] = f32x4{0.f, 0.f, 0.f, 0.f};
    }

    f32x16 acc_m, acc_c;
#pragma unroll
    for (int r = 0; r < 16; r++) { acc_m[r] = 0.f; acc_c[r] = 0.f; }
    const int a_off = kg * 32 + l31;
    const bool w_exact = p.w_exact != 0;
    const int b_off = (wv * S * PCL + l31) * PXB + kg * 16;
    auto compute = [&]() {
#pragma unroll
        for (int t = 0; t < TAPS; t++) {
            if (!((tap_mask >> t) & 1u)) continue;
            const int r = t / KW, s = t % KW;
            const int col = S == 2 ? (s & 1) * Cfg::PCH + (s >> 1) : s;
            const char* bp = sIn + b_off + (r * PCL + col) * PXB;
            const f16x8 bh = *reinterpret_cast<const f16x8*>(bp);
            const f16x8 ah = __builtin_bit_cast(f16x8, sW[a_off + (t * 2 + 0) * 64]);
            acc_m = __builtin_amdgcn_mfma_f32_32x32x16_f16(ah, bh, acc_m, 0, 0, 0);
            if (!w_exact) {
                const f16x8 al = __builtin_bit_cast(f16x8, sW[a_off + (t * 2 + 1) * 64]);
                acc_c = __builtin_amdgcn_mfma_f32_32x32x16_f16(al, bh, acc_c, 0, 0, 0);
            }
            if constexpr (!XF16) {
                const f16x8 bl = *reinterpret_cast<const f16x8*>(bp + 32);
                acc_c = __builtin_amdgcn_mfma_f32_32x32x16_f16(ah, bl, acc_c, 0, 0, 0);
            }
        }
    };

    if (kgi < nchunks) prefetch(kgi);
    RT_TSTAMP();
    for (int ch = kgi; ch < nchunks + kgi; ch += KS) {
        const bool mine = KS == 1 || ch < nchunks;
        if (ch != kgi) __syncthreads();
        if (mine) stage_to_lds();
        __syncthreads();
        RT_TSTAMP();
        if (ch + KS < nchunks) prefetch(ch + KS);
        if (mine) compute();
        RT_TSTAMP();
    }

#pragma unroll
    for (int r = 0; r < 16; r++) acc_m[r] = fmaf(acc_c[r], kSplitInv, acc_m[r]);
    if (KS > 1) {
        f32x4* const red = reinterpret_cast<f32x4*>(smem);
        __syncthreads();
        if (kgi > 0) {
#pragma unroll
            for (int q = 0; q < 4; q++)
                red[(((kgi - 1) * NW + wv) * 4 + q) * 64 + lane] = f32x4{acc_m[4 * q], acc_m[4 * q + 1], acc_m[4 * q + 2], acc_m[4 * q + 3]};
        }
        __syncthreads();
        if (kgi > 0) return;
        for (int g = 1; g < KS; g++)
#pragma unroll
            for (int q = 0; q < 4; q++) {
                const f32x4 v = red[(((g - 1) * NW + wv) * 4 + q) * 64 + lane];
#pragma unroll
                for (int e = 0; e < 4; e++) acc_m[4 * q + e] += v[e];
            }
    }

    const buf_rsrc rs_y = make_buf(elem_ptr(p.y, (YIL && !YF16) ? (int64_t)n * p.y_bstride + y_off_il4 : ybase, ESY));
    auto epilogue = [&](auto ACT) {
#pragma unroll
        for (int q = 0; q < 4; q++) {
            const f32x4 bv = *reinterpret_cast<const f32x4*>(p.bias + cb + 8 * q + 4 * kg);
            f32x4 o;
#pragma unroll
            for (int e = 0; e < 4; e++)
                o[e] = apply_act_fast(acc_m[4 * q + e] + (bv[e] + rr[q][e]), decltype(ACT)::value);
            if constexpr (YIL && YF16) {
                const unsigned vo = (inb && cb + 8 * q + 4 * kg < p.Cout) ? (unsigned)((oy * p.y_ystride + ox * p.y_xstride) * 8 + 4 * kg) * 2u : kBufOOB;
                u32x2_t w2;
#pragma unroll
                for (int e = 0; e < 2; e++)
                    w2[e] = (unsigned)__builtin_bit_cast(unsigned short, (_Float16)o[2 * e]) | ((unsigned)__builtin_bit_cast(unsigned short, (_Float16)o[2 * e + 1]) << 16);
                __builtin_amdgcn_raw_buffer_store_b64(w2, rs_y, vo, (unsigned)((cb + 8 * q) * cs32) * 2u, 0);
            } else if constexpr (YIL) {
                const unsigned vo = (inb && cb + 8 * q + 4 * kg < p.Cout) ? (unsigned)((oy * p.y_ystride + ox * p.y_xstride) * 4 + 4 * kg * cs32) * 4u : kBufOOB;
                buf_store4(o, rs_y, vo, (unsigned)((cb + 8 * q) * cs32) * 4u);
            } else {
                const unsigned vo = inb ? (unsigned)(oy * p.y_ystride + ox * p.y_xstride + 4 * kg * cs32) * ESY : kBufOOB;
#pragma unroll
                for (int e = 0; e < 4; e++)
                    Io<TOUT>::store(o[e], rs_y, (cb + 8 * q + 4 * kg + e < p.Cout) ? vo : kBufOOB, (unsigned)((cb + 8 * q + e) * cs32) * ESY);
            }
        }
    };
    if (act == 1) epilogue(std::integral_constant<int, 1>{});
    else if (act == 2) epilogue(std::integral_constant<int, 2>{});
    else epilogue(std::integral_constant<int, 0>{});
    RT_TSTAMP();
#ifdef RT_KERNEL_TIMING
    __builtin_amdgcn_s_waitcnt(0);
    if (dbgp && tid == 0) { dbgp[14] = __builtin_amdgcn_s_memtime(); dbgp[15] = __builtin_amdgcn_s_memrealtime() - rt0; }
#endif
}

}

namespace rt {

struct S3FirstCfg {
    static constexpr int KH = 5, KW = 5, S = 2, TY = 4, TX = 32, CMAX = 3;
    static constexpr int PR = (TY - 1) * S + KH, PC = (TX - 1) * S + KW;
    static constexpr int NPAIR = (PC + 1) / 2;
    static constexpr int RS = 208;
    static constexpr int NRUN = NPAIR / 2, NRUN_T = PR * NRUN;
    static_assert(NPAIR % 2 == 0 && NRUN_T <= 256 && (RS * 2) % 8 == 0 && NRUN * 4 * CMAX <= RS, "one gather per lane, 8-byte LDS writes");
    static constexpr int W_SLOTS = KH * 2 * 2 * 32;
};

template <bool YIL>
__global__ void __launch_bounds__(256) RT_WAVES_PER_EU(4) conv_s3_first_kernel(ConvArgs p) {
    using Cfg = S3FirstCfg;
    constexpr int KH = Cfg::KH, S = Cfg::S, TY = Cfg::TY, TX = Cfg::TX, PR = Cfg::PR, RS = Cfg::RS;

    __shared__ __attribute__((aligned(16))) _Float16 sHi[PR * RS];
    __shared__ __attribute__((aligned(16))) _Float16 sLo[PR * RS];

    const int tid = threadIdx.x;
    const int lane = tid & 63;
    const int kg = lane >> 5, l31 = lane & 31;
    const int wv = __builtin_amdgcn_readfirstlane(tid >> 6);

    int tile = blockIdx.x;
    if (p.xcd_order) {
        const int nwg = gridDim.x, q = nwg >> 3, r = nwg & 7;
        const int xcd = blockIdx.x & 7, idx = blockIdx.x >> 3;
        tile = (xcd < r ? xcd * (q + 1) : r * (q + 1) + (xcd - r) * q) + idx;
    }
    const int tx0 = (tile % p.tiles_x) * TX;
    const int ty0 = (tile / p.tiles_x) * TY;
    const int nblk = blockIdx.y;
    const int n = blockIdx.z;

    f32x4 wa[KH][2];
    {
        const buf_rsrc rs_w = make_buf(reinterpret_cast<const char*>(p.w) + (int64_t)nblk * Cfg::W_SLOTS * 16);
#pragma unroll
        for (int r = 0; r < KH; r++)
#pragma unroll
            for (int part = 0; part < 2; part++) wa[r][part] = buf_load4(rs_w, (unsigned)(((r * 2 + part) * 2 + kg) * 32 + l31) * 16u, 0);
    }

    const int cb = nblk * 32;
    f32x4 bv[4];
#pragma unroll
    for (int q = 0; q < 4; q++) bv[q] = *reinterpret_cast<const f32x4*>(p.bias + cb + 8 * q + 4 * kg);

    const buf_rsrc rs_x = make_buf((p.x2 && n >= p.x2_from) ? p.x2 + (int64_t)(n - p.x2_from) * p.x_bstride : p.x + (int64_t)n * p.x_bstride);
    const int ix0 = tx0 * S - p.pad_x, iy0 = ty0 * S - p.pad_y;
    const int cin = p.cin_real;
    if (tid < Cfg::NRUN_T) {
// ... 330 lines not shown
```

redtail_amd/csrc/rt_capi.hip:

```cpp
#include <hip/hip_runtime.h>

#include <algorithm>
#include <atomic>
#include <cmath>
#include <cstdarg>
#include <cstdio>
#include <cstdlib>
#include <cstring>
#include <string>
#include <map>
#include <mutex>
#include <vector>

#include "../../include/rt_stereo.h"
#if defined(__HIP_DEVICE_COMPILE__) && !defined(RT_BUILT_NO_SLP)
#error "rt_capi.hip must be compiled with -fno-slp-vectorize -DRT_BUILT_NO_SLP (redtail_amd/build.py: DEVICE_FLAGS)"
#endif
#include "kernels/common.hip.h"
#include "kernels/conv_mfma.hip.h"
#include "kernels/conv_wino.hip.h"
#include "kernels/deconv3d_small.hip.h"
#include "kernels/imgproc.hip.h"
#include "kernels/rectify.hip.h"
#include "kernels/decode.hip.h"
// ... 1204 lines not shown
    int TY = 4, TXW = 2, NW = 4, WLDS = 1;
    int CinPad = 0, Cout = 0;
    int Hi = 0, Wi = 0, Ho = 0, Wo = 0, pad_y = 0, pad_x = 0, nz = 1;
    int x_pitch = 0;
    std::vector<rt::ZSlice> zs_host;
    int64_t y_cstride = 0, y_zstride = 0, y_off = 0;
    int64_t r_cstride = 0;
    int y_ystride = 0, y_xstride = 1;
    float* w_dev = nullptr;
    int* choff_dev = nullptr;
    int w_exact = 0;
    int* shift_dev = nullptr;
    rt::ZSlice* zs_dev = nullptr;
    int direct = 0, cin_real = 0;
    int wino = 0;
    int x_f16 = 0, y_f16 = 0;
    int f16mma = 0;
    int x_il8 = 0, y_il8 = 0, r_il8 = 0;
    int dp4 = 0;
    int f16first = 0;
    int split3 = 0;
    int rb = 0;
    int s3first = 0;
    int s3p = 0;
    int small3d = 0;
    rt::Deconv3dSmallArgs s3{};
    std::vector<float> small_w;
    void* small_il_dev = nullptr;
    int small_il_f32 = 0;
};

}

struct FoldFactor {
    rtConvPlan* pl = nullptr;
    rtConvPlan* pr = nullptr;
    float* wedge_dev = nullptr;
    int F = 0, K = 0, D = 0, H = 0, W = 0;
    int64_t a_elems = 0, c_elems = 0, t_elems = 0, e_elems = 0;
    std::mutex mu;
    std::map<rtStream, std::pair<void*, size_t>> own;
};

struct ConvKnobs {
    int xcd = 1, trace = 0;
    int rb_tiles = 0;
    int rbs_seg = 0;
    int ksplit = -1;
    int s3p_grid = 0;
    int zinner = 1;
    int nbinner = 1;
    int dw = -1;
    int dw_nseg = 0;
    int fold_u = 2;
    int f16p_walk = -1;
    int f16p_classes = 1;
    int small_walk = -1;
    int r4 = -1;
};

struct rtConvPlan {
    std::vector<SubConv> subs;
    FoldFactor* ff = nullptr;
    mutable std::once_flag env_once;
    mutable ConvKnobs opt;
    int softarg = 0;
    float* bias_dev = nullptr;
    float* zeros_dev = nullptr;
    int act = 0, has_resid = 0, dtype = RT_F32;
    int out_dims[4] = {0, 0, 0, 1};
    int64_t x_bstride = 0, y_bstride = 0;
    int64_t r_bstride = 0;
    int is2d = 0, cin = 0, hin = 0, win = 0;
    std::vector<float> w_canon;
    rtConv2dDesc desc2d{};
    int is_deconv = 0;
    int in_pitch = 0, out_pitch = 0;
    float* rb_w1_dev = nullptr;
    float* rb_bias1_dev = nullptr;
    int rb_act1 = 0, rb_cmid = 0;
    float* rbd_w1_dev = nullptr;
    float* rbd_w2_dev = nullptr;
    int x_split = 0, y_split = 0;
    float* rbh_w1_dev = nullptr;
    float* rbh_w2_dev = nullptr;
    int w_f16 = 0;
    int is_conv3d = 0, is_deconv3d = 0;
    int c3d_C = 0, c3d_cin = 0, c3d_dchw = 0, c3d_fold = 0;
    int c3d_dw = 0;
    rtConv3dDesc desc3d{};
    int in_dims3[3] = {0, 0, 0};
    int flags = 0;
};

namespace {

struct Phase1D {
    int K = 0;
    int pad = 0;
    int tap[8] = {0};
};
Phase1D phase1d(int s, int p, int k, int phi) {
    Phase1D ph;
    int r0 = -1;
    for (int r = k - 1; r >= 0; r--)
        if (((r - (phi + p)) % s + s) % s == 0) { r0 = r; break; }
    if (r0 < 0) return ph;
    ph.pad = -((phi + p - r0) / s);
    for (int r = r0; r >= 0; r -= s) ph.tap[ph.K++] = r;
    return ph;
}

void split_f16(float w, uint16_t& hi, uint16_t& lo) {
    const _Float16 h = (_Float16)w;
    const _Float16 l = (_Float16)((w - (float)h) * rt::kSplitScale);
    std::memcpy(&hi, &h, 2);
    std::memcpy(&lo, &l, 2);
}

template <typename F>
int64_t pack_into(std::vector<float>& packed, const SubConv& sc, int cin_real, F wfun) {
    const int64_t base = (int64_t)packed.size();
    const int taps = sc.KH * sc.KW;
    if (sc.direct) {
        packed.resize(base + (size_t)sc.Cout * cin_real * taps, 0.f);
        for (int co = 0; co < sc.Cout; co++)
            for (int ci = 0; ci < cin_real; ci++)
                for (int u = 0; u < sc.KH; u++)
                    for (int v = 0; v < sc.KW; v++)
                        packed[base + ((size_t)co * cin_real + ci) * taps + u * sc.KW + v] = wfun(co, ci, u, v);
        return base;
    }
    if (sc.split3) {
        const int nblk = (int)rt::cdiv(sc.Cout, 32), nch = sc.CinPad / 16;
        const size_t slots = (size_t)nblk * nch * taps * 2 * 2 * 32;
        packed.resize(base + slots * 4, 0.f);
        uint16_t* dst = reinterpret_cast<uint16_t*>(packed.data() + base);
        for (int co = 0; co < sc.Cout; co++)
            for (int ci = 0; ci < cin_real; ci++)
                for (int u = 0; u < sc.KH; u++)
                    for (int v = 0; v < sc.KW; v++) {
                        uint16_t hi, lo;
                        split_f16(wfun(co, ci, u, v), hi, lo);
                        const int nb = co / 32, cc = co % 32, ch = ci / 16, kg = (ci % 16) / 8, e = ci % 8, t = u * sc.KW + v;
                        const size_t slab = ((size_t)nb * nch + ch) * taps + t;
                        dst[(((slab * 2 + 0) * 2 + kg) * 32 + cc) * 8 + e] = hi;
                        dst[(((slab * 2 + 1) * 2 + kg) * 32 + cc) * 8 + e] = lo;
                    }
        return base / 4;
    }
    if (sc.wino) {
        static const double G[4][3] = {{1, 0, 0}, {.5, .5, .5}, {.5, -.5, .5}, {0, 0, 1}};
        const int nblk = (int)rt::cdiv(sc.Cout, 32), nch = sc.CinPad / 8;
        packed.resize(base + (size_t)nblk * nch * 4096, 0.f);
        for (int co = 0; co < sc.Cout; co++)
            for (int ci = 0; ci < cin_real; ci++) {
                double g[3][3], tmp[4][3];
                for (int u = 0; u < 3; u++)
                    for (int v = 0; v < 3; v++) g[u][v] = wfun(co, ci, u, v);
                for (int a = 0; a < 4; a++)
                    for (int v = 0; v < 3; v++) tmp[a][v] = G[a][0] * g[0][v] + G[a][1] * g[1][v] + G[a][2] * g[2][v];
                const int nb = co / 32, cc = co % 32, ch = ci / 8, j = (ci % 8) / 4, k4 = ci % 4;
                for (int pr = 0; pr < 4; pr++)
                    for (int pc = 0; pc < 4; pc++) {
                        const double u = tmp[pr][0] * G[pc][0] + tmp[pr][1] * G[pc][1] + tmp[pr][2] * G[pc][2];
                        const int pp = 4 * pr + pc;
// ... 145 lines not shown
    if (sc.KH == 5) sc.CC = 4;
    const int forced = env_int("RT_CONV_VARIANT", -1);
    set_tile(sc, forced >= 0 ? forced : 6);
    sc.wino = (allow_wino && !sc.direct && sc.KH == 3 && sc.KW == 3 && sc.S == 1 && sc.Cout >= 24 && env_int("RT_CONV_NO_WINO", 0) == 0) ? 1 : 0;
    if (sc.wino) { sc.CC = 8; sc.NBW = 1; sc.TY = exp_knob("RT_WINO_WAVES", 4); sc.TXW = 1; sc.NW = sc.TY; }
    const int nbw = env_int("RT_CONV_NBW", 0);
    if (nbw == 1 || (nbw == 2 && sc.KH != 5)) sc.NBW = nbw;
    const bool s3_win = (sc.KH == 3 && sc.KW == 3 && (sc.S == 1 || sc.S == 2)) || (sc.S == 1 && sc.KH <= 2 && sc.KW <= 2);
    sc.split3 = (!sc.direct && s3_win && !exact_fp32() && env_int("RT_NO_S3", 0) == 0) ? 1 : 0;
    if (sc.split3) {
        sc.wino = 0; sc.CC = 16; sc.NBW = 1; sc.TY = 4; sc.TXW = 1; sc.NW = 4;
        if (sc.KH == 3 && sc.KW == 3 && sc.S == 1 && exp_knob("RT_S3_ROWS", 4) == 8) sc.TY = sc.NW = 8;
    }
}

bool s3p_eligible(const SubConv& sc, int cin) {
    return !sc.direct && sc.KH == 3 && sc.KW == 3 && sc.S == 1 && cin <= 32 && sc.Cout <= 32 && sc.nz == 1 &&
           !exact_fp32() && exp_knob("RT_S3P", 0) != 0;
}

template <typename F>
int upload_s3p(SubConv& sc, int cin_real, F wfun) {
    std::vector<uint16_t> packed((size_t)rt::S3PCfg<8>::W_SLOTS * 8, 0);
    for (int co = 0; co < sc.Cout; co++)
        for (int ci = 0; ci < cin_real; ci++)
            for (int t = 0; t < 9; t++) {
                uint16_t hi, lo;
                split_f16(wfun(co, ci, t / 3, t % 3), hi, lo);
                const int c = ci / 16, kg = (ci % 16) / 8, e = ci % 8;
                packed[(((((size_t)t * 2 + c) * 2 + 0) * 2 + kg) * 32 + co) * 8 + e] = hi;
                packed[(((((size_t)t * 2 + c) * 2 + 1) * 2 + kg) * 32 + co) * 8 + e] = lo;
            }
    if (int rc = upload_weights(sc, packed)) return rc;
    sc.s3p = 1; sc.split3 = 0; sc.wino = 0;
    sc.CinPad = 32; sc.CC = 16; sc.NBW = 1; sc.TXW = 1; sc.TY = sc.NW = 8;
    return 0;
}

bool s3first_eligible(const SubConv& sc, int cin, int has_resid) {
    return !sc.direct && sc.KH == 5 && sc.KW == 5 && sc.S == 2 && cin <= 3 && !has_resid && sc.nz == 1 &&
           !exact_fp32() && env_int("RT_NO_S3", 0) == 0;
}
template <typename F>
int upload_s3first(SubConv& sc, int cin_real, F wfun) {
    const int nblk = (int)rt::cdiv(sc.Cout, 32);
    std::vector<uint16_t> packed((size_t)nblk * rt::S3FirstCfg::W_SLOTS * 8, 0);
    for (int co = 0; co < sc.Cout; co++)
        for (int c = 0; c < cin_real; c++)
            for (int r = 0; r < 5; r++)
                for (int sx = 0; sx < 5; sx++) {
                    uint16_t hi, lo;
                    split_f16(wfun(co, c, r, sx), hi, lo);
                    const int k = 3 * sx + c, h = k / 8, e = k % 8;
                    const size_t blk = (size_t)(co / 32) * rt::S3FirstCfg::W_SLOTS * 8;
                    packed[blk + ((((size_t)r * 2 + 0) * 2 + h) * 32 + co % 32) * 8 + e] = hi;
                    packed[blk + ((((size_t)r * 2 + 1) * 2 + h) * 32 + co % 32) * 8 + e] = lo;
                }
    if (int rc = upload_weights(sc, packed)) return rc;
    sc.s3first = 1; sc.s3p = 0; sc.split3 = 0; sc.wino = 0;
    sc.NBW = 1; sc.TXW = 1; sc.TY = sc.NW = 4;
    return 0;
}

template <bool Z, int PAT>
bool drop_structural_zeros(std::vector<float>& packed) {
    using Taps = rt::SmallTaps<Z, PAT>;
    constexpr int NJ = Taps::NJ;
    if (env_int("RT_NO_SMALL_SPARSE", 0) != 0) return false;
    const size_t rows = packed.size() / (NJ * NJ);
    for (size_t r = 0; r < rows; r++)
        for (int f = 0; f < NJ; f++)
            for (int j = 0; j < NJ; j++)
                if (!Taps::valid(f, j) && packed[(r * NJ + f) * NJ + j] != 0.f) return false;
    std::vector<float> dense(rows * Taps::NV);
    for (size_t r = 0; r < rows; r++)
        for (int f = 0; f < NJ; f++)
            for (int j = 0; j < NJ; j++)
                if (Taps::valid(f, j)) dense[r * Taps::NV + Taps::index(f, j)] = packed[(r * NJ + f) * NJ + j];
    packed.swap(dense);
    return true;
}

template <typename T> constexpr const char* type_tag() { return sizeof(T) == 2 ? "f16" : "f32"; }
template <int KH, int KW, int S, bool XIL, bool YIL, int NW = 4, typename TIN = float, typename TOUT = float>
void launch_s3(dim3 grid, int ks, int64_t per_cu, hipStream_t st, const rt::ConvArgs& a, int trace = 0) {
    using Cfg = rt::S3Cfg<KH, KW, S, NW>;
    ks = Cfg::max_groups(ks);
    while (ks > 1 && std::min<int64_t>(per_cu, 4) * ks * Cfg::GRP_BYTES > 160 * 1024) ks = Cfg::max_groups(ks - 1);
    if (trace)
        fprintf(stderr, "[rt] conv_s3<%d,%d,%d,%d,%d,%d,%s,%s> r%d grid %u x %u x %u ks %d\n", KH, KW, S, (int)XIL, (int)YIL, NW, type_tag<TIN>(),
                type_tag<TOUT>(), a.r_il8, grid.x, grid.y, grid.z, ks);
#ifndef HIPEMU
    static std::atomic<unsigned long long> done{0};
    int dev = 0;
    if (hipGetDevice(&dev) == hipSuccess && dev >= 0 && dev < 64 && !((done.load(std::memory_order_acquire) >> dev) & 1ull)) {
        (void)hipFuncSetAttribute(reinterpret_cast<const void*>(&rt::conv_s3_kernel<KH, KW, S, XIL, YIL, NW, TIN, TOUT>),
                                  hipFuncAttributeMaxDynamicSharedMemorySize, Cfg::KS_MAX * Cfg::GRP_BYTES);
        done.fetch_or(1ull << dev, std::memory_order_release);
    }
#endif
    hipLaunchKernelGGL((rt::conv_s3_kernel<KH, KW, S, XIL, YIL, NW, TIN, TOUT>), grid, dim3(64 * NW * ks), (size_t)ks * Cfg::GRP_BYTES, st, a);
}

int device_cus() {
    static std::atomic<int> cus[64];
    int dev = 0;
    if (hipGetDevice(&dev) != hipSuccess || dev < 0 || dev >= 64) return 256;
    int n = cus[dev].load(std::memory_order_relaxed);
    if (!n) {
        hipDeviceProp_t prop;
        n = (hipGetDeviceProperties(&prop, dev) == hipSuccess && prop.multiProcessorCount > 0) ? prop.multiProcessorCount : 256;
        cus[dev].store(n, std::memory_order_relaxed);
    }
    return n;
}

std::vector<float> to_f32(const void* w, size_t n, int dtype) {
    std::vector<float> out(n);
    if (dtype == RT_F16) {
        const char* h = static_cast<const char*>(w);
        for (size_t i = 0; i < n; i++) {
            _Float16 v;
            std::memcpy(&v, h + 2 * i, 2);
            out[i] = (float)v;
        }
    } else {
        std::memcpy(out.data(), w, n * sizeof(float));
    }
    return out;
}

template <int KH, int KW, int S, int NBW, int CC>
int launch_window(const SubConv& sc, const rt::ConvArgs& a, dim3 grid, hipStream_t st) {
#define RT_TILE(ty, txw, nw, wlds)                                                                        \
    if (sc.TY == ty && sc.TXW == txw && sc.NW == nw && sc.WLDS == (wlds ? 1 : 0)) {                       \
        hipLaunchKernelGGL((rt::conv_mfma_f32_kernel<KH, KW, S, ty, txw, NBW, CC, nw, wlds>), grid,       \
                           dim3(64 * nw), 0, st, a);                                                      \
        return 0;                                                                                         \
    }
    if (sc.y_il8) return 1;
    if (sc.x_f16 || sc.y_f16) {
        if (!(sc.TY == 4 && sc.TXW == 1 && sc.NW == 4 && sc.WLDS) || !sc.y_f16) return 1;
        if (sc.x_f16)
            hipLaunchKernelGGL((rt::conv_mfma_f32_kernel<KH, KW, S, 4, 1, NBW, CC, 4, true, _Float16, _Float16>), grid, dim3(256), 0, st, a);
        else
            hipLaunchKernelGGL((rt::conv_mfma_f32_kernel<KH, KW, S, 4, 1, NBW, CC, 4, true, float, _Float16>), grid, dim3(256), 0, st, a);
        return 0;
    }
    RT_TILE(4, 2, 4, true) RT_TILE(4, 1, 4, true) RT_TILE(2, 2, 4, true) RT_TILE(2, 1, 2, true) RT_TILE(8, 1, 8, true) RT_TILE(8, 1, 4, true)
#undef RT_TILE
    return 1;
}

int launch_sub(const SubConv& sc, const rt::ConvArgs& a, dim3 grid, hipStream_t st) {
#define RT_CASE(kh, kw, s, nbw, cc)                                                             \
    if (sc.KH == kh && sc.KW == kw && sc.S == s && sc.NBW == nbw && sc.CC == cc) {              \
        if (launch_window<kh, kw, s, nbw, cc>(sc, a, grid, st))                                 \
            return fail(RT_E_UNSUPPORTED, "conv: tile %dx%d/%d waves not instantiated", sc.TY, 32 * sc.TXW, sc.NW); \
        RT_LAUNCH_CHECK("conv_mfma_f32_kernel<" #kh "," #kw "," #s "," #nbw "," #cc ">");       \
        return 0;                                                                               \
    }
    RT_CASE(3, 3, 1, 1, 8) RT_CASE(3, 3, 1, 2, 8)
    RT_CASE(3, 3, 2, 1, 8) RT_CASE(3, 3, 2, 2, 8)
    RT_CASE(5, 5, 2, 1, 4)
    RT_CASE(1, 1, 1, 1, 8) RT_CASE(1, 1, 1, 2, 8)
    RT_CASE(1, 2, 1, 1, 8) RT_CASE(1, 2, 1, 2, 8)
    RT_CASE(2, 1, 1, 1, 8) RT_CASE(2, 1, 1, 2, 8)
    RT_CASE(2, 2, 1, 1, 8) RT_CASE(2, 2, 1, 2, 8)
#undef RT_CASE
    return fail(RT_E_UNSUPPORTED, "conv: no kernel for window %dx%d stride %d", sc.KH, sc.KW, sc.S);
}

void free_subs(rtConvPlan* p) {
    for (auto& s : p->subs) {
        if (s.w_dev) (void)hipFree(s.w_dev);
        if (s.choff_dev) (void)hipFree(s.choff_dev);
        if (s.shift_dev) (void)hipFree(s.shift_dev);
        if (s.zs_dev) (void)hipFree(s.zs_dev);
        if (s.small_il_dev) (void)hipFree(s.small_il_dev);
    }
    p->subs.clear();
}

void free_plan(rtConvPlan* p) {
// ... 95 lines not shown
    sc.y_cstride = (int64_t)sc.Ho * sc.Wo; sc.y_ystride = sc.Wo; sc.y_xstride = 1;
    sc.cin_real = d1->Cin; sc.CinPad = 32; sc.CC = 16;
    const std::vector<float> wa = to_f32(w1, (size_t)d1->Cout * d1->Cin * 9, d1->dtype), wb = to_f32(w2, (size_t)d2->Cout * d2->Cin * 9, d2->dtype);
    const int c1 = d1->Cin, c2 = d2->Cin;
    sc.split3 = 1;
    SubConv tmp = sc;
    tmp.Cout = d1->Cout;
    int rc = upload_packed(tmp, c1, [&](int co, int ci, int u, int v) { return wa[(((size_t)co * c1 + ci) * 3 + u) * 3 + v]; });
    plan->rb_w1_dev = tmp.w_dev;
    if (!rc) rc = upload_packed(sc, c2, [&](int co, int ci, int u, int v) { return wb[(((size_t)co * c2 + ci) * 3 + u) * 3 + v]; });
    sc.split3 = 0; sc.rb = 1; sc.TY = 4; sc.NW = 4; sc.TXW = 1; sc.NBW = 1;
    std::vector<int> table(sc.CinPad, -1);
    for (int c = 0; c < c1; c++) table[c] = c * d1->Hin * d1->Win;
    if (!rc) rc = upload_table(sc, table);
    plan->subs.push_back(sc);
    if (!rc) {
        const std::vector<float> bb = b2 ? to_f32(b2, d2->Cout, d2->dtype) : std::vector<float>();
        rc = upload_bias(plan, b2 ? bb.data() : nullptr, d2->Cout);
    }
    if (!rc) {
        std::vector<float> ba(64, 0.f);
        if (b1) { const std::vector<float> t = to_f32(b1, d1->Cout, d1->dtype); std::copy(t.begin(), t.end(), ba.begin()); }
        if (hipMalloc((void**)&plan->rb_bias1_dev, ba.size() * 4) != hipSuccess ||
            hipMemcpy(plan->rb_bias1_dev, ba.data(), ba.size() * 4, hipMemcpyHostToDevice) != hipSuccess)
            rc = fail(RT_E_NOMEM, "rt_resblock_plan_create: device allocation failed");
    }
    if (!rc && d1->Cin == 32 && d1->Cout == 32 && d2->Cout == 32) {
        auto rbd_row = [](int co) { return 8 * (2 * (co >> 4) + ((co >> 2) & 1)) + 4 * ((co >> 3) & 1) + (co & 3); };
        auto pack = [&](const std::vector<float>& w, float** dev) {
            std::vector<uint16_t> slab((size_t)18 * 2 * 64 * 8, 0);
            for (int co = 0; co < 32; co++)
                for (int ci = 0; ci < 32; ci++)
                    for (int t = 0; t < 9; t++) {
                        uint16_t hi, lo;
                        split_f16(w[((size_t)co * 32 + ci) * 9 + t], hi, lo);
                        const size_t sl = (size_t)(ci / 16) * 9 + t;
                        const int kg = (ci % 16) / 8, e = ci % 8, row = rbd_row(co);
                        slab[(((sl * 2 + 0) * 2 + kg) * 32 + row) * 8 + e] = hi;
                        slab[(((sl * 2 + 1) * 2 + kg) * 32 + row) * 8 + e] = lo;
                    }
            if (hipMalloc((void**)dev, slab.size() * 2) != hipSuccess || hipMemcpy(*dev, slab.data(), slab.size() * 2, hipMemcpyHostToDevice) != hipSuccess)
                return fail(RT_E_NOMEM, "rt_resblock_plan_create: device allocation failed");
            return 0;
        };
        rc = pack(wa, &plan->rbd_w1_dev);
        if (!rc) rc = pack(wb, &plan->rbd_w2_dev);
        auto pack16 = [&](const std::vector<float>& w, float** dev) {
            std::vector<uint16_t> slab((size_t)18 * 64 * 8, 0);
            for (int co = 0; co < 32; co++)
                for (int ci = 0; ci < 32; ci++)
                    for (int t = 0; t < 9; t++) {
                        const _Float16 hv = (_Float16)w[((size_t)co * 32 + ci) * 9 + t];
                        const size_t sl = (size_t)(ci / 16) * 9 + t;
                        std::memcpy(&slab[((sl * 2 + (ci % 16) / 8) * 32 + rbd_row(co)) * 8 + ci % 8], &hv, 2);
                    }
            if (hipMalloc((void**)dev, slab.size() * 2) != hipSuccess || hipMemcpy(*dev, slab.data(), slab.size() * 2, hipMemcpyHostToDevice) != hipSuccess)
                return fail(RT_E_NOMEM, "rt_resblock_plan_create: device allocation failed");
            return 0;
        };
        if (!rc) rc = pack16(wa, &plan->rbh_w1_dev);
        if (!rc) rc = pack16(wb, &plan->rbh_w2_dev);
    }
    if (rc) { free_plan(plan); return rc; }
    *out = plan;
    return 0;
}

extern "C" int rt_resblock_plan_supports_split(const rtConvPlan* plan);
extern "C" int rt_resblock_plan_set_split(rtConvPlan* plan, int x_split, int y_split) {
    RT_REQUIRE(plan, "rt_resblock_plan_set_split: null plan");
    if (!x_split && !y_split) { plan->x_split = plan->y_split = 0; return 0; }
    if (!rt_resblock_plan_supports_split(plan))
        return fail(RT_E_UNSUPPORTED, "rt_resblock_plan_set_split: only the tower block takes pre-split tensors (32 -> 32 -> 32 channels, ELU after both "
                                       "convolutions, fp32 channel-interleaved tensors: call rt_conv_plan_set_layouts(1, 1, 1) first)");
    plan->x_split = x_split != 0; plan->y_split = y_split != 0;
    return 0;
}

extern "C" int rt_resblock_plan_supports_split(const rtConvPlan* plan) {
    if (!plan || plan->subs.size() != 1 || !plan->rbd_w1_dev || env_int("RT_NO_RBD", 0) != 0) return 0;
    const SubConv& sc = plan->subs[0];
    return sc.rb && sc.x_il8 && sc.y_il8 && !sc.x_f16 && !sc.y_f16 && plan->cin == 32 && plan->rb_cmid == 32 && sc.Cout == 32 && plan->rb_act1 == 1 &&
           plan->act == 1 && !(plan->flags & RT_CONV_EXACT_FP32);
}

extern "C" int rt_deconv2d_plan_create(rtConvPlan** out, const rtConv2dDesc* d, const void* weights, const void* bias) {
    ExactScope exact_scope(d ? d->flags : 0);
    RT_REQUIRE(out && d && weights, "rt_deconv2d_plan_create: null pointer");
    RT_REQUIRE(d->Cin > 0 && d->Cout > 0 && d->Hin > 0 && d->Win > 0, "rt_deconv2d_plan_create: bad dims");
    RT_REQUIRE(d->dtype == RT_F32 || d->dtype == RT_F16, "rt_deconv2d_plan_create: bad dtype");
    if (!((d->KH == 3 && d->KW == 3) || (d->KH == 1 && d->KW == 1)) || d->stride < 1 || d->stride > 2)
        return fail(RT_E_UNSUPPORTED, "deconv2d: only 3x3 / 1x1 kernels with stride 1 or 2");
    const int s = d->stride;
    const int Ho = (d->Hin - 1) * s - 2 * d->pad_h + d->KH;
    const int Wo = (d->Win - 1) * s - 2 * d->pad_w + d->KW;
    RT_REQUIRE(Ho > 0 && Wo > 0, "deconv2d: empty output");
    RT_REQUIRE((int64_t)d->Cin * d->Hin * d->Win < (1ll << 29), "deconv2d: input sample exceeds 2 GB (32-bit buffer offsets)");

    auto plan = new rtConvPlan();
    plan->act = d->act; plan->has_resid = d->has_residual; plan->dtype = RT_F32; plan->w_f16 = d->dtype == RT_F16;
    plan->out_dims[0] = d->Cout; plan->out_dims[1] = Ho; plan->out_dims[2] = Wo; plan->out_dims[3] = 1;
    plan->x_bstride = (int64_t)d->Cin * d->Hin * d->Win;
    plan->y_bstride = (int64_t)d->Cout * Ho * Wo;
    plan->is2d = 1; plan->cin = d->Cin; plan->hin = d->Hin; plan->win = d->Win;
    plan->desc2d = *d; plan->is_deconv = 1; plan->flags = d->flags;
    const std::vector<float> w = to_f32(weights, (size_t)d->Cin * d->Cout * d->KH * d->KW, d->dtype);
    plan->w_canon = w;
    const int Cin = d->Cin, Cout = d->Cout, KH = d->KH, KW = d->KW;

    if (Cout <= 2 && KH == 3 && KW == 3 && s == 2 && env_int("RT_NO_DECONV3D_SMALL", 0) == 0) {
        const Phase1D qy[2] = {phase1d(2, d->pad_h, 3, 0), phase1d(2, d->pad_h, 3, 1)};
        const Phase1D qx[2] = {phase1d(2, d->pad_w, 3, 0), phase1d(2, d->pad_w, 3, 1)};
        auto base_of = [](const Phase1D* ph, bool& ok) {
            int lo = 1 << 20, hi = -(1 << 20);
            for (int f = 0; f < 2; f++)
                for (int u = 0; u < ph[f].K; u++) { lo = std::min(lo, u - ph[f].pad); hi = std::max(hi, u - ph[f].pad); }
            ok = ok && hi - lo <= 1;
            return lo;
        };
        bool ok = true;
        const int by = base_of(qy, ok), bx = base_of(qx, ok);
        if (ok) {
            std::vector<float> packed((size_t)Cin * Cout * 16, 0.f);
            for (int k = 0; k < Cin; k++)
                for (int co = 0; co < Cout; co++)
                    for (int fy = 0; fy < 2; fy++)
                        for (int fx = 0; fx < 2; fx++)
                            for (int uy = 0; uy < qy[fy].K; uy++)
                                for (int ux = 0; ux < qx[fx].K; ux++) {
                                    const int jy = uy - qy[fy].pad - by, jx = ux - qx[fx].pad - bx;
                                    packed[(((size_t)k * Cout + co) * 4 + 2 * fy + fx) * 4 + 2 * jy + jx] +=
                                        w[(((size_t)k * Cout + co) * KH + qy[fy].tap[uy]) * KW + qx[fx].tap[ux]];
                                }
            SubConv sc;
            sc.small3d = 2; sc.Cout = Cout; sc.nz = 1;
            sc.s3.K = Cin; sc.s3.Dy = 1; sc.s3.Hy = d->Hin; sc.s3.Wy = d->Win;
            sc.s3.Dx = 1; sc.s3.Hx = Ho; sc.s3.Wx = Wo; sc.s3.C = Cout;
            sc.s3.bz = 0; sc.s3.by = by; sc.s3.bx = bx; sc.s3.Mz = 1;
            sc.s3.xp = d->Win; sc.s3.yp = Wo;
            sc.s3.sparse = (by == 0 && bx == 0 && drop_structural_zeros<false, 0>(packed)) ? 1 : 0;
            int rc = upload_weights(sc, packed);
            plan->subs.push_back(sc);
            if (!rc) {
                const std::vector<float> b = bias ? to_f32(bias, Cout, d->dtype) : std::vector<float>();
                rc = upload_bias(plan, bias ? b.data() : nullptr, Cout);
            }
            if (rc) { free_plan(plan); return rc; }
            *out = plan;
            return 0;
        }
    }
    std::vector<Phase1D> py_ph, px_ph;
    int wy = 1, wx = 1;
    for (int ph = 0; ph < s; ph++) {
        py_ph.push_back(phase1d(s, d->pad_h, KH, ph));
        px_ph.push_back(phase1d(s, d->pad_w, KW, ph));
        wy = std::max(wy, py_ph.back().K);
        wx = std::max(wx, px_ph.back().K);
    }
    SubConv sc;
    sc.KH = wy; sc.KW = wx; sc.S = 1; sc.Cout = Cout; sc.Hi = d->Hin; sc.Wi = d->Win;
    sc.Ho = (Ho + s - 1) / s; sc.Wo = (Wo + s - 1) / s;
    sc.y_cstride = (int64_t)Ho * Wo; sc.y_ystride = s * Wo; sc.y_xstride = s;
    sc.nz = 0;
    for (int py = 0; py < s; py++)
        for (int px = 0; px < s; px++)
// ... 767 lines not shown
        }
        if (sc.split3 && !xf && yf && sc.KH == 3 && sc.KW == 3 && sc.S == 1 && !plan->is_deconv && !plan->has_resid && sc.TY == 4) {
            sc.x_f16 = 0; sc.y_f16 = 1;
            continue;
        }
        if (sc.rb && xf && yf && plan->rbh_w1_dev && plan->cin == 32 && plan->rb_cmid == 32 && sc.Cout == 32 && plan->rb_act1 == 1 && plan->act == 1 &&
            env_int("RT_NO_F16MMA", 0) == 0 && env_int("RT_NO_RBH", 0) == 0) {
            sc.x_f16 = sc.y_f16 = 1;
            continue;
        }
        if (sc.s3p || sc.split3 || sc.s3first || sc.rb) return fail(RT_E_UNSUPPORTED, "rt_conv_plan_set_io_types: the split-fp16 kernels take fp32 tensors (both fp16: fp16 operands instead)");
        if (sc.small3d) { if (!(sc.small3d == 2 && xf)) return fail(RT_E_UNSUPPORTED, "rt_conv_plan_set_io_types: unsupported combination for the small-output kernel"); }
        else if (sc.wino) { if (!(xf && yf)) return fail(RT_E_UNSUPPORTED, "rt_conv_plan_set_io_types: Winograd layers take fp16 on both sides"); }
        else if (!yf) return fail(RT_E_UNSUPPORTED, "rt_conv_plan_set_io_types: fp16 -> fp32 is only built for the small-output kernel");
        else set_tile(sc, 6);
        sc.x_f16 = xf; sc.y_f16 = yf;
    }
    return 0;
}

extern "C" int rt_conv_plan_supports_il8(const rtConvPlan* plan) {
    if (!plan) return 0;
    ExactScope exact_scope(plan->flags);
    if (!plan->is2d) {
        if (env_int("RT_NO_IL8", 0) != 0 || env_int("RT_NO_IL8_3D", 0) != 0 || plan->subs.empty()) return 0;
        const SubConv& sc = plan->subs[0];
        if (plan->is_conv3d && plan->subs.size() == 1 && plan->ff && !sc.x_f16 && !sc.f16mma)
            return 32 | 2;
        if (plan->is_conv3d && plan->subs.size() == 1) {
            const int out_dm = (plan->c3d_dchw && sc.Cout % 8 == 0) ? 2 : 0, out = sc.Cout % 8 == 0 ? 2 : 0;
            const bool f16mma_ok = !sc.small3d && !sc.direct && (sc.split3 || sc.f16mma) && sc.KH == 3 && sc.KW == 3 &&
                                   (sc.S == 1 || sc.S == 2) && sc.TY == 4 && plan->c3d_C % 8 == 0 && env_int("RT_NO_F16MMA_3D", 0) == 0;
            if (sc.x_f16 && sc.y_f16) return f16mma_ok ? (1 | out | (out ? 8 : 0) | ((out && plan->has_resid) ? 4 : 0)) : 0;
            if (sc.split3 && sc.y_f16 && !sc.x_f16 && sc.TY == 4) return out_dm;
            if (sc.split3 && !sc.x_f16 && !sc.y_f16 && sc.TY == 4 && sc.KH == 3 && sc.KW == 3 && env_int("RT_NO_IL8_3D_F32", 0) == 0) {
                const int o4 = (plan->c3d_dchw && sc.Cout % 4 == 0) ? 2 : 0;
                return ((plan->c3d_C % 4 == 0 && plan->c3d_fold % 4 == 0) ? 1 : 0) | o4 | ((o4 && plan->has_resid) ? 4 : 0);
            }
            return 0;
        }
        if (plan->is_deconv3d) {
            if (sc.small3d) {
                if (sc.small3d != 1 || sc.y_f16 || sc.s3.K % 32 != 0 || sc.small_w.empty() || env_int("RT_NO_SMALL_IL", 0) != 0) return 0;
                if (!sc.x_f16 && ((plan->flags & RT_CONV_EXACT_FP32) || env_int("RT_NO_IL8_3D_F32", 0) != 0 || env_int("RT_NO_SMALL_IL_F32", 0) != 0)) return 0;
                return 1;
            }
            bool all_f32 = true;
            for (const SubConv& q : plan->subs) all_f32 = all_f32 && q.split3 && !q.x_f16 && !q.y_f16 && q.TY == 4;
            if (all_f32) {
                if (plan->c3d_C % 4 != 0 || env_int("RT_NO_IL8_3D_F32", 0) != 0) return 0;
                return (plan->has_resid ? 4 : 0) | (sc.dp4 ? 2 : 0);
            }
            for (const SubConv& q : plan->subs)
                if (!(q.split3 || q.f16mma) || !q.y_f16 || q.TY != 4) return 0;
            const bool f16mma_ok = sc.x_f16 && ((sc.KH == 2 && sc.KW == 2) || sc.dp4) && plan->desc3d.K % 8 == 0 && env_int("RT_NO_F16MMA_3D", 0) == 0 &&
                                   env_int("RT_NO_DECONV_IL", 0) == 0;
            int caps = (plan->has_resid && plan->c3d_C % 8 == 0) ? 4 : 0;
            if (f16mma_ok) caps |= 1 | (plan->c3d_C % 8 == 0 ? 2 | 8 : 0);
            return caps;
        }
        return 0;
    }
    if (plan->subs.size() != 1) return 0;
    if (plan->subs[0].split3 && env_int("RT_NO_IL8", 0) == 0) {
        if (plan->subs[0].y_f16) return (plan->cin % 4 == 0 ? 1 : 0) | (plan->subs[0].Cout % 8 == 0 ? 2 : 0);
        return (plan->cin % 4 == 0 ? 1 : 16) | (plan->subs[0].Cout % 4 == 0 ? 6 : 0);
    }
    if (plan->is_deconv) return 0;
    const SubConv& sc = plan->subs[0];
    if (env_int("RT_NO_IL8", 0) != 0 || sc.zs_dev || sc.y_xstride != 1 || sc.small3d || sc.direct) return 0;
    if (sc.s3p) return (plan->cin % 4 == 0 ? 1 : 0) | (sc.Cout % 4 == 0 ? 6 : 0);
    if (sc.rb) return (plan->cin % 4 == 0 ? 5 : 0) | (sc.Cout % 4 == 0 ? 2 : 0);
    if (sc.s3first) return sc.Cout % 4 == 0 ? 2 : 0;
    if (sc.f16first) return sc.Cout % 8 == 0 ? 2 : 0;
    if (sc.f16mma) return (sc.KH == 3 && sc.KW == 3 && sc.S == 1 && sc.Cout % 8 == 0) ? ((plan->cin % 8 == 0 ? 1 : 16) | 6) : 0;
    if (sc.x_f16 || sc.y_f16) return 0;
    if (sc.wino) return (env_int("RT_NO_WINO_IL8", 0) == 0 && sc.TY == 4 && plan->cin % 4 == 0 && sc.Cout % 4 == 0) ? 7 : 0;
    return 0;
}
extern "C" int rt_conv_plan_set_layouts(rtConvPlan* plan, int x_il8, int y_il8, int r_il8) {
    RT_REQUIRE(plan, "rt_conv_plan_set_layouts: null plan");
    ExactScope exact_scope(plan->flags);
    struct KeepOnFailure {
        rtConvPlan* p; int softarg, xs, ys; bool ok = false;
        ~KeepOnFailure() { if (!ok) { p->softarg = softarg; p->x_split = xs; p->y_split = ys; } }
    } keep{plan, plan->softarg, plan->x_split, plan->y_split};
    plan->softarg = 0;
    plan->x_split = plan->y_split = 0;
    if (!x_il8 && !y_il8 && !r_il8) {
        if (plan->is_conv3d && plan->subs.size() == 1 && plan->subs[0].f16mma)
            if (int rc = switch_conv3d_f16mma(plan, false)) return rc;
        if (plan->is_deconv3d && !plan->subs.empty() && plan->subs[0].f16mma) {
            const int xf = plan->subs[0].x_f16, yf = plan->subs[0].y_f16;
            if (int rc = build_deconv3d_subs(plan, false, !xf && !yf && deconv3d_p4f32_ok(plan))) return rc;
            for (SubConv& q : plan->subs) { q.x_f16 = xf; q.y_f16 = yf; }
        }
        for (SubConv& sc : plan->subs) sc.x_il8 = sc.y_il8 = sc.r_il8 = 0;
        keep.ok = true;
        return 0;
    }
    const int caps = rt_conv_plan_supports_il8(plan);
    if (plan->is_conv3d && plan->subs.size() == 1 && plan->subs[0].x_f16 && plan->subs[0].y_f16) {
        if ((caps & 8) && y_il8 && !x_il8) return fail(RT_E_UNSUPPORTED, "rt_conv_plan_set_layouts: this Conv3D writes an interleaved tensor only when it reads one");
        if ((x_il8 && !(caps & 1)) || (y_il8 && !(caps & 2))) return fail(RT_E_UNSUPPORTED, "rt_conv_plan_set_layouts: this Conv3D plan takes no interleaved tensors");
        if (r_il8 && (!(caps & 4) || !x_il8)) return fail(RT_E_UNSUPPORTED, "rt_conv_plan_set_layouts: this Conv3D reads an interleaved skip tensor only on fp16 operands (interleaved input)");
        if (int rc = switch_conv3d_f16mma(plan, x_il8 != 0)) return rc;
        SubConv& sc = plan->subs[0];
        sc.x_il8 = x_il8 != 0; sc.y_il8 = y_il8 != 0; sc.r_il8 = r_il8 != 0;
        keep.ok = true;
        return 0;
    }
    if (plan->is_deconv3d && !plan->subs.empty()) {
        if ((x_il8 && !(caps & 1)) || (y_il8 && !(caps & 2)) || (r_il8 && !(caps & 4)) || ((caps & 8) && y_il8 && !x_il8))
            return fail(RT_E_UNSUPPORTED, "rt_conv_plan_set_layouts: this Conv3DTranspose plan does not take that combination of interleaved tensors (caps %d)", caps);
        RT_REQUIRE(!r_il8 || plan->has_resid, "rt_conv_plan_set_layouts: plan has no residual");
        if (plan->subs[0].small3d) {
            SubConv& sc = plan->subs[0];
            const bool f32in = !sc.x_f16;
            if (x_il8 && sc.small_il_dev && sc.small_il_f32 != (f32in ? 1 : 0)) { (void)hipFree(sc.small_il_dev); sc.small_il_dev = nullptr; }
            if (x_il8 && !sc.small_il_dev && f32in) {
                const int K = sc.s3.K, CO = sc.Cout, KC = K / 32;
                std::vector<uint16_t> slab((size_t)2 * 8 * KC * 64 * 8, 0);
                for (int j = 0; j < 8; j++)
                    for (int kc = 0; kc < KC; kc++)
                        for (int l = 0; l < 64; l++)
                            for (int e = 0; e < 8; e++) {
                                const int row = l % 16, co = row / 8, f = row % 8, k = kc * 32 + 8 * (l / 16) + e;
                                if (co >= CO) continue;
                                uint16_t hi, lo;
                                split_f16(sc.small_w[(((size_t)k * CO + co) * 8 + f) * 8 + j], hi, lo);
                                slab[(((size_t)j * KC + kc) * 64 + l) * 8 + e] = hi;
                                slab[(((size_t)(8 + j) * KC + kc) * 64 + l) * 8 + e] = lo;
                            }
                RT_HIP(hipMalloc(&sc.small_il_dev, slab.size() * 2));
                RT_HIP(hipMemcpy(sc.small_il_dev, slab.data(), slab.size() * 2, hipMemcpyHostToDevice));
                sc.small_il_f32 = 1;
            }
            if (x_il8 && !sc.small_il_dev) {
                sc.small_il_f32 = 0;
                const int K = sc.s3.K, CO = sc.Cout, KC = K / 32;
                std::vector<uint16_t> slab((size_t)8 * KC * 64 * 8, 0);
                for (int j = 0; j < 8; j++)
                    for (int kc = 0; kc < KC; kc++)
                        for (int l = 0; l < 64; l++)
                            for (int e = 0; e < 8; e++) {
                                const int row = l % 16, co = row / 8, f = row % 8, k = kc * 32 + 8 * (l / 16) + e;
                                if (co >= CO) continue;
                                const _Float16 h = (_Float16)sc.small_w[(((size_t)k * CO + co) * 8 + f) * 8 + j];
                                std::memcpy(&slab[(((size_t)j * KC + kc) * 64 + l) * 8 + e], &h, 2);
                            }
                RT_HIP(hipMalloc(&sc.small_il_dev, slab.size() * 2));
                RT_HIP(hipMemcpy(sc.small_il_dev, slab.data(), slab.size() * 2, hipMemcpyHostToDevice));
            }
            sc.x_il8 = x_il8 != 0;
            keep.ok = true;
            return 0;
        }
        const bool f32 = !plan->subs[0].x_f16 && !plan->subs[0].y_f16;
        const bool want = x_il8 != 0, want_dp = want ? (y_il8 && deconv3d_dp4_ok(plan)) : (f32 && deconv3d_p4f32_ok(plan));
        if ((plan->subs[0].f16mma != 0) != want || (plan->subs[0].dp4 != 0) != want_dp) {
            const int xf = plan->subs[0].x_f16, yf = plan->subs[0].y_f16;
            if (int rc = build_deconv3d_subs(plan, want, want_dp)) return rc;
            for (SubConv& q : plan->subs) { q.x_f16 = xf; q.y_f16 = yf; }
        }
        for (SubConv& q : plan->subs) { q.x_il8 = x_il8 != 0; q.y_il8 = y_il8 != 0; q.r_il8 = r_il8 != 0; }
        keep.ok = true;
        return 0;
    }
    if ((x_il8 && !(caps & (1 | 16))) || (y_il8 && !(caps & 2)) || (r_il8 && !(caps & 4)))
        return fail(RT_E_UNSUPPORTED, "rt_conv_plan_set_layouts: this plan does not take an interleaved %s tensor (3x3 stride-1 plans take all three; "
                    "the first layer and stride-2 3x3 layers write one; channel counts must be multiples of 4 in fp32, 8 in fp16)",
// ... 129 lines not shown
            else hipLaunchKernelGGL((rt::deconv3d_s2_small_kernel<2, false, _Float16, float>), grid, dim3(256), 0, S(L.s), a);
        }
    } else if (sc.small3d == 1 && sc.x_f16 && sc.x_il8) {
        a.w = static_cast<const float*>(sc.small_il_dev);
        const int groups = (int)rt::cdiv((a.Wx + 1) / 2, 16);
        RT_REQUIRE(batch <= 65535, "rt_conv_enqueue: grid limit exceeded");
        const int rowpairs = (int)rt::cdiv((a.Hx + 1) / 2, 2);
        if (plan->softarg) {
            RT_REQUIRE(a.K == 32 && a.C == 1 && !a.resid && rowpairs <= 65535, "rt_conv_enqueue: plan lost the form its fused soft-argmax needs");
            a.y_bstride = (int64_t)a.Hx * a.Wx;
            dim3 gw((unsigned)rt::cdiv(groups, 4), (unsigned)rowpairs, (unsigned)batch);
            if (plan->opt.trace) fprintf(stderr, "[rt] deconv3d_s2_ilw<%d> grid %u x %u x %u segments 1 x %d\n", plan->softarg == 2 ? 2 : 1, gw.x, gw.y, gw.z, a.Mz);
            if (plan->softarg == 2) hipLaunchKernelGGL(rt::deconv3d_s2_ilw_kernel<2>, gw, dim3(256), 0, S(L.s), a, a.Mz, 1);
            else hipLaunchKernelGGL(rt::deconv3d_s2_ilw_kernel<1>, gw, dim3(256), 0, S(L.s), a, a.Mz, 1);
        } else if (a.K == 32 && plan->opt.small_walk != 0) {
            const int64_t waves = (int64_t)groups * rowpairs * batch;
            int nseg = (int)std::min<int64_t>(std::max<int64_t>(1, rt::cdiv((int64_t)8 * device_cus(), waves)), std::max(1, a.Mz / 8));
            const int seg_len = (int)rt::cdiv(a.Mz, nseg);
            nseg = (int)rt::cdiv(a.Mz, seg_len);
            RT_REQUIRE(rowpairs <= 65535, "rt_conv_enqueue: grid limit exceeded");
            dim3 gw((unsigned)(rt::cdiv(groups, 4) * nseg), (unsigned)rowpairs, (unsigned)batch);
            if (plan->opt.trace) fprintf(stderr, "[rt] deconv3d_s2_ilw<0> grid %u x %u x %u segments %d x %d\n", gw.x, gw.y, gw.z, nseg, seg_len);
            hipLaunchKernelGGL(rt::deconv3d_s2_ilw_kernel<0>, gw, dim3(256), 0, S(L.s), a, seg_len, nseg);
        } else {
            dim3 g2((unsigned)(rt::cdiv(groups, 4 * rt::kSmallIlIters) * a.Mz), (unsigned)rowpairs, (unsigned)batch);
            if (plan->opt.trace) fprintf(stderr, "[rt] deconv3d_s2_il grid %u x %u x %u\n", g2.x, g2.y, g2.z);
            hipLaunchKernelGGL(rt::deconv3d_s2_il_kernel, g2, dim3(256), 0, S(L.s), a);
        }
    } else if (sc.small3d == 1 && !sc.x_f16 && sc.x_il8) {
        RT_REQUIRE(sc.small_il_dev && sc.small_il_f32, "rt_conv_enqueue: interleaved fp32 input without its weight operands (rt_conv_plan_set_layouts)");
        a.w = static_cast<const float*>(sc.small_il_dev);
        const int groups = (int)rt::cdiv((a.Wx + 1) / 2, 16);
        RT_REQUIRE(batch <= 65535, "rt_conv_enqueue: grid limit exceeded");
        dim3 g2((unsigned)(rt::cdiv(groups, 4 * rt::kSmallIlIters) * a.Mz), (unsigned)rt::cdiv((a.Hx + 1) / 2, 2), (unsigned)batch);
        if (plan->opt.trace) fprintf(stderr, "[rt] deconv3d_s2_il4 grid %u x %u x %u\n", g2.x, g2.y, g2.z);
        hipLaunchKernelGGL(rt::deconv3d_s2_il4_kernel, g2, dim3(256), 0, S(L.s), a);
    } else if (sc.small3d == 1 && sc.x_f16) {
        if (a.C == 1) hipLaunchKernelGGL((rt::deconv3d_s2_small_kernel<1, true, _Float16, float>), grid, dim3(256), 0, S(L.s), a);
        else hipLaunchKernelGGL((rt::deconv3d_s2_small_kernel<2, true, _Float16, float>), grid, dim3(256), 0, S(L.s), a);
    } else if (sc.small3d == 2) {
        if (a.C == 1) hipLaunchKernelGGL((rt::deconv3d_s2_small_kernel<1, false>), grid, dim3(256), 0, S(L.s), a);
        else hipLaunchKernelGGL((rt::deconv3d_s2_small_kernel<2, false>), grid, dim3(256), 0, S(L.s), a);
    } else {
        if (a.C == 1) hipLaunchKernelGGL((rt::deconv3d_s2_small_kernel<1, true>), grid, dim3(256), 0, S(L.s), a);
        else hipLaunchKernelGGL((rt::deconv3d_s2_small_kernel<2, true>), grid, dim3(256), 0, S(L.s), a);
    }
    RT_LAUNCH_CHECK("deconv3d_s2_small_kernel");
    return 0;
}

rt::ConvArgs conv_args(const Launch& L, const SubConv& sc) {
    const rtConvPlan* plan = L.plan;
    rt::ConvArgs a;
    a.z_inner = 0; a.nb_inner = 0;
    a.x = static_cast<const float*>(L.x);
    a.x2 = static_cast<const float*>(L.x2); a.x2_from = L.x2_from;
    a.y = static_cast<float*>(L.y);
    a.w = sc.w_dev;
    a.bias = plan->bias_dev;
    a.zeros = plan->zeros_dev;
    a.dbg = nullptr;
#ifdef RT_KERNEL_TIMING
    if (const char* e = getenv("RT_DBG_PTR")) a.dbg = (unsigned long long*)strtoull(e, nullptr, 0);
#endif
    a.resid = plan->has_resid ? static_cast<const float*>(L.residual) : nullptr;
    a.ch_off = sc.choff_dev;
    a.ch_shift = sc.shift_dev;
    a.w_exact = plan->w_f16;
    a.zs = sc.zs_dev;
    a.CinPad = sc.CinPad; a.Cout = sc.Cout;
    a.Hi = sc.Hi; a.Wi = sc.Wi; a.Ho = sc.Ho; a.Wo = sc.Wo;
    a.x_pitch = sc.x_pitch ? sc.x_pitch : sc.Wi;
    a.pad_y = sc.pad_y; a.pad_x = sc.pad_x; a.nz = sc.nz;
    a.tiles_x = (int)rt::cdiv(sc.Wo, 32 * sc.TXW);
    a.act = plan->act;
    a.xcd_order = plan->opt.xcd;
    a.x_bstride = plan->x_bstride; a.y_bstride = plan->y_bstride;
    a.y_cstride = sc.y_cstride; a.y_zstride = sc.y_zstride; a.y_off = sc.y_off;
    if (plan->is_conv3d && !plan->c3d_dchw && sc.y_il8) a.y_zstride = 8 * sc.y_zstride;
    a.y_ystride = sc.y_ystride; a.y_xstride = sc.y_xstride;
    a.r_cstride = sc.r_cstride ? sc.r_cstride : sc.y_cstride;
    a.r_bstride = plan->r_bstride ? plan->r_bstride : plan->y_bstride;
    a.r_il8 = sc.r_il8;
    a.batch = L.batch; a.cin_real = sc.cin_real; a.x_cstride = (int64_t)sc.Hi * a.x_pitch;
    return a;
}

int enqueue_deconv_s3p(const Launch& L, const SubConv& sc, rt::ConvArgs& a) {
    a.tiles_x = (int)rt::cdiv(sc.Wi, 32);
    const int tiles = a.tiles_x * (int)rt::cdiv(sc.Hi, 4), nblk = (int)rt::cdiv(sc.Cout, 32);
    RT_REQUIRE(!sc.x_il8 && !sc.x_f16 && !sc.y_f16, "rt_conv_enqueue: the fp32 four-phase transposed kernel takes a planar fp32 input and writes fp32");
    RT_REQUIRE((int64_t)L.batch * sc.nz <= 65535, "rt_conv_enqueue: grid limit exceeded");
    RT_REQUIRE(sc.y_cstride * (int64_t)sc.Cout < (1ll << 29), "rt_conv_enqueue: output sample exceeds 2 GB (32-bit buffer offsets)");
    dim3 g((unsigned)tiles, (unsigned)nblk, (unsigned)(L.batch * sc.nz));
    if (L.plan->opt.trace) fprintf(stderr, "[rt] deconv_s3p<%d> r%d grid %u x %u x %u\n", sc.y_il8 ? 1 : 0, sc.r_il8, g.x, g.y, g.z);
    if (sc.y_il8) hipLaunchKernelGGL(rt::deconv_s3p_kernel<true>, g, dim3(256), 0, S(L.s), a);
    else hipLaunchKernelGGL(rt::deconv_s3p_kernel<false>, g, dim3(256), 0, S(L.s), a);
    RT_LAUNCH_CHECK("deconv_s3p_kernel");
    return 0;
}

int enqueue_deconv_f16p(const Launch& L, const SubConv& sc, rt::ConvArgs& a, bool& took_next) {
    const rtConvPlan* plan = L.plan;
    const int batch = L.batch;
    a.tiles_x = (int)rt::cdiv(sc.Wi, 32);
    const int tiles = a.tiles_x * (int)rt::cdiv(sc.Hi, 4), nblk = (int)rt::cdiv(sc.Cout, 32);
    RT_REQUIRE(sc.x_il8 && sc.y_il8 && sc.x_f16 && sc.y_f16, "rt_conv_enqueue: the four-phase transposed kernel takes interleaved fp16 tensors");
    a.z_inner = plan->opt.zinner != 0 ? 1 : 0;
    RT_REQUIRE(batch <= 65535 && (int64_t)batch * sc.nz <= 65535, "rt_conv_enqueue: grid limit exceeded");
    dim3 g = a.z_inner ? dim3((unsigned)(tiles * sc.nz), (unsigned)nblk, (unsigned)batch) : dim3((unsigned)tiles, (unsigned)nblk, (unsigned)(batch * sc.nz));
    if (plan->opt.f16p_walk != 0 && (!plan->has_resid || sc.r_il8)) {
        rt::DeconvWalkB wb{};
        const SubConv* sb = (&sc == &plan->subs[0] && plan->subs.size() == 2) ? &plan->subs[1] : nullptr;
        if (sb && plan->opt.f16p_classes != 0 && sb->dp4 && sb->f16mma && sb->x_il8 && sb->y_il8 && sb->x_f16 && sb->y_f16 && sb->r_il8 == sc.r_il8 &&
            sb->Hi == sc.Hi && sb->Wi == sc.Wi && sb->Ho == sc.Ho && sb->Wo == sc.Wo && sb->Cout == sc.Cout && sb->x_pitch == sc.x_pitch &&
            sb->y_cstride == sc.y_cstride && sb->y_ystride == sc.y_ystride && sb->r_cstride == sc.r_cstride) {
            wb.w = static_cast<const float*>(sb->w_dev); wb.zs = sb->zs_dev; wb.ch_off = sb->choff_dev; wb.CinPad = sb->CinPad; wb.nz = sb->nz;
            took_next = true;
        }
        const int nzw = std::max(sc.nz, wb.zs ? wb.nz : 0);
        const double per_m = wb.zs ? (double)(sc.CinPad + wb.CinPad) / sc.CinPad : 1.0;
        const int64_t slots = (int64_t)3 * device_cus(), base = (int64_t)tiles * nblk * batch;
        int nseg = 1;
        double best = 1e30;
        auto seg_cost = [&](int ns) {
            const int seg = (int)rt::cdiv(nzw, ns);
            return (int)rt::cdiv(nzw, seg) != ns ? 1e30 : (double)rt::cdiv(base * ns, slots) * (seg * per_m + 1.0);
        };
        for (int ns = 1; ns <= nzw; ns++) best = std::min(best, seg_cost(ns));
        for (int ns = 1; ns <= nzw; ns++)
            if (seg_cost(ns) <= 1.05 * best) nseg = ns;
        if (plan->opt.f16p_walk > 0) nseg = std::min(plan->opt.f16p_walk, nzw);
        a.dw_seg = (int)rt::cdiv(nzw, nseg); a.dw_nseg = nzw; a.dw_cpc = sc.nz; a.nz = (int)rt::cdiv(nzw, a.dw_seg);
        RT_REQUIRE((int64_t)batch * a.nz <= 65535, "rt_conv_enqueue: grid limit exceeded");
        dim3 gw = a.z_inner ? dim3((unsigned)(tiles * a.nz), (unsigned)nblk, (unsigned)batch) : dim3((unsigned)tiles, (unsigned)nblk, (unsigned)(batch * a.nz));
        if (plan->opt.trace) fprintf(stderr, "[rt] deconv_f16pw grid %u x %u x %u, %d slice indices per segment, %d class(es)\n", gw.x, gw.y, gw.z, a.dw_seg, wb.zs ? 2 : 1);
        hipLaunchKernelGGL(rt::deconv_f16pw_kernel, gw, dim3(256), 0, S(L.s), a, wb);
        RT_LAUNCH_CHECK("deconv_f16pw_kernel");
        return 0;
    }
    if (plan->opt.trace) fprintf(stderr, "[rt] deconv_f16p grid %u x %u x %u\n", g.x, g.y, g.z);
    hipLaunchKernelGGL(rt::deconv_f16p_kernel, g, dim3(256), 0, S(L.s), a);
    RT_LAUNCH_CHECK("deconv_f16p_kernel");
    return 0;
}

struct ConvGrid {
    dim3 grid;
    int64_t gz = 0;
    unsigned nz_fold = 0, batch = 0;
    int tiles_y = 0, nb_fold = 0;
    dim3 fold(dim3 g) const {
        if (nz_fold) g = dim3(g.x * nz_fold, g.y, batch);
        return nb_fold ? dim3(g.x * g.y, 1u, g.z) : g;
    }
};

int conv_grid(const Launch& L, const SubConv& sc, rt::ConvArgs& a, ConvGrid& g) {
    const rtConvPlan* plan = L.plan;
    g.tiles_y = (int)rt::cdiv(sc.Ho, sc.TY);
    g.gz = (int64_t)L.batch * sc.nz;
    g.batch = (unsigned)L.batch;
    const bool zin = sc.nz > 1 && plan->opt.zinner != 0 && (sc.f16mma || (sc.split3 && plan->opt.zinner == 2)) &&
                     (int64_t)rt::cdiv(sc.Wo, 32 * sc.TXW) * rt::cdiv(sc.Ho, sc.TY) * sc.nz < (1ll << 30);
    a.z_inner = zin ? 1 : 0;
    g.nz_fold = zin ? (unsigned)sc.nz : 0u;
// ... 55 lines not shown
        seg = seg < 4 ? 4 : (seg > 240 ? 240 : (seg + 3) / 4 * 4);
        ra.seg = seg;
        dim3 sgrid((unsigned)(ra.c.tiles_x * (int)rt::cdiv(sc.Ho, seg)), 1u, (unsigned)L.batch);
        if (plan->opt.trace) {
            if (sc.x_f16) fprintf(stderr, "[rt] conv_f16rbd grid %u x %u x %u seg %d\n", sgrid.x, sgrid.y, sgrid.z, seg);
            else fprintf(stderr, "[rt] conv_s3rb%c<%d> grid %u x %u x %u seg %d\n", plan->x_split ? 'd' : 's', plan->y_split ? 1 : 0, sgrid.x,
                         sgrid.y, sgrid.z, seg);
        }
        if (sc.x_f16) {
            ra.w1 = plan->rbh_w1_dev; ra.c.w = plan->rbh_w2_dev;
            hipLaunchKernelGGL(rt::conv_f16rbd_kernel, sgrid, dim3(512), 0, S(L.s), ra);
            RT_LAUNCH_CHECK("conv_f16rbd_kernel");
        } else if (plan->x_split) {
            ra.w1 = plan->rbd_w1_dev; ra.c.w = plan->rbd_w2_dev;
            if (plan->y_split) hipLaunchKernelGGL(rt::conv_s3rbd_kernel<true>, sgrid, dim3(512), 0, S(L.s), ra);
            else hipLaunchKernelGGL(rt::conv_s3rbd_kernel<false>, sgrid, dim3(512), 0, S(L.s), ra);
            RT_LAUNCH_CHECK("conv_s3rbd_kernel");
        } else {
            if (plan->y_split) hipLaunchKernelGGL(rt::conv_s3rbs_kernel<true>, sgrid, dim3(512), 0, S(L.s), ra);
            else hipLaunchKernelGGL(rt::conv_s3rbs_kernel<false>, sgrid, dim3(512), 0, S(L.s), ra);
            RT_LAUNCH_CHECK("conv_s3rbs_kernel");
        }
        return 0;
    }
    if (sc.x_f16 || sc.y_f16)
        return fail(RT_E_UNSUPPORTED, "rt_conv_enqueue: the half2 form of the residual block takes channel-interleaved fp16 tensors only (rt_conv_plan_set_layouts(1, 1, 1))");
#ifdef RT_EXPERIMENTAL
    dim3 rgrid((unsigned)(a.tiles_x * g.tiles_y), 1u, (unsigned)L.batch);
    if (plan->opt.trace) fprintf(stderr, "[rt] conv_s3rb x%d y%d grid %u x %u\n", sc.x_il8, sc.y_il8, rgrid.x, rgrid.z);
    with_bools([&](auto xi, auto yi) { hipLaunchKernelGGL((rt::conv_s3rb_kernel<xi, yi>), rgrid, dim3(256), 0, S(L.s), ra); }, sc.x_il8, sc.y_il8);
    RT_LAUNCH_CHECK("conv_s3rb_kernel");
    return 0;
#else
    return fail(RT_E_UNSUPPORTED, "rt_conv_enqueue: this build plans residual blocks for the streaming kernel only (32 -> 32 -> 32 channels, "
                                   "ELU / ELU, interleaved tensors); the per-tile form is compiled with RT_EXPERIMENTAL");
#endif
}

int enqueue_s3first(const Launch& L, const SubConv& sc, const rt::ConvArgs& a, const ConvGrid& g) {
    if (L.plan->opt.trace) fprintf(stderr, "[rt] conv_s3_first<%d> grid %u x %u x %u twin %d\n", sc.y_il8 ? 1 : 0, g.grid.x, g.grid.y, g.grid.z, a.x2 ? 1 : 0);
    if (sc.y_il8) hipLaunchKernelGGL((rt::conv_s3_first_kernel<true>), g.grid, dim3(256), 0, S(L.s), a);
    else hipLaunchKernelGGL((rt::conv_s3_first_kernel<false>), g.grid, dim3(256), 0, S(L.s), a);
    RT_LAUNCH_CHECK("conv_s3_first_kernel");
    return 0;
}

int enqueue_f16first(const Launch& L, const SubConv& sc, const rt::ConvArgs& a, const ConvGrid& g) {
    if (L.plan->opt.trace) fprintf(stderr, "[rt] conv_f16_first<%d> grid %u x %u x %u twin %d\n", sc.y_il8 ? 1 : 0, g.grid.x, g.grid.y, g.grid.z, a.x2 ? 1 : 0);
    if (sc.y_il8) hipLaunchKernelGGL((rt::conv_f16_first_kernel<true>), g.grid, dim3(256), 0, S(L.s), a, L.plan->cin);
    else hipLaunchKernelGGL((rt::conv_f16_first_kernel<false>), g.grid, dim3(256), 0, S(L.s), a, L.plan->cin);
    RT_LAUNCH_CHECK("conv_f16_first_kernel");
    return 0;
}

int enqueue_split3(const Launch& L, const SubConv& sc, const rt::ConvArgs& a, const ConvGrid& g) {
    const rtConvPlan* plan = L.plan;
    const dim3 grid = g.fold(g.grid);
    const int trace = plan->opt.trace;
    bool launched = false;
    int ks = 1;
    const int64_t per_cu = rt::cdiv((int64_t)g.grid.x * g.grid.y * (g.gz / L.batch), (int64_t)device_cus());
    if (plan->opt.ksplit > 0 || (plan->opt.ksplit < 0 && !(L.hints & RT_HINT_THROUGHPUT))) {
        const int nch = a.CinPad / 16;
        ks = plan->opt.ksplit > 0 ? plan->opt.ksplit : (per_cu == 1 && nch >= 4 ? 4 : (per_cu <= 2 && nch >= 2 ? 2 : 1));
    }
    if (sc.x_f16 || sc.y_f16) {
        if (!sc.x_f16 && sc.x_il8 && sc.KH == 3 && sc.KW == 3 && sc.S == 1 && sc.TY == 4 && sc.y_f16) {
            if (sc.y_il8) launch_s3<3, 3, 1, true, true, 4, float, _Float16>(grid, ks, per_cu, S(L.s), a, trace);
            else launch_s3<3, 3, 1, true, false, 4, float, _Float16>(grid, ks, per_cu, S(L.s), a, trace);
            RT_LAUNCH_CHECK("conv_s3_kernel<float, f16>");
            return 0;
        }
        RT_REQUIRE(!sc.x_il8 && !(sc.y_il8 && sc.x_f16) && sc.TY == 4 && sc.y_f16, "rt_conv_enqueue: fp16-storage variant of the split kernel not instantiated");
#define RT_S3H(kh, kw, st)                                                                                           \
    if (!launched && sc.KH == kh && sc.KW == kw && sc.S == st) {                                                     \
        if (sc.x_f16) launch_s3<kh, kw, st, false, false, 4, _Float16, _Float16>(grid, ks, per_cu, S(L.s), a, trace); \
        else if (sc.y_il8) launch_s3<kh, kw, st, false, true, 4, float, _Float16>(grid, ks, per_cu, S(L.s), a, trace); \
        else launch_s3<kh, kw, st, false, false, 4, float, _Float16>(grid, ks, per_cu, S(L.s), a, trace);            \
        launched = true;                                                                                             \
    }
        RT_S3H(3, 3, 1) RT_S3H(3, 3, 2) RT_S3H(1, 1, 1) RT_S3H(1, 2, 1) RT_S3H(2, 1, 1) RT_S3H(2, 2, 1)
#undef RT_S3H
    }
#ifdef RT_EXPERIMENTAL
    if (!launched && sc.KH == 3 && sc.KW == 3 && sc.S == 1 && sc.TY == 8) {
        with_bools([&](auto xi, auto yi) { launch_s3<3, 3, 1, xi, yi, 8>(grid, ks, per_cu, S(L.s), a, trace); }, sc.x_il8, sc.y_il8);
        launched = true;
    }
#endif
#define RT_S3(kh, kw, st)                                                                                                              \
    if (!launched && sc.KH == kh && sc.KW == kw && sc.S == st) {                                                                       \
        with_bools([&](auto xi, auto yi) { launch_s3<kh, kw, st, xi, yi>(grid, ks, per_cu, S(L.s), a, trace); }, sc.x_il8, sc.y_il8); \
        launched = true;                                                                                                               \
    }
    RT_S3(3, 3, 1) RT_S3(3, 3, 2) RT_S3(1, 1, 1) RT_S3(1, 2, 1) RT_S3(2, 1, 1) RT_S3(2, 2, 1)
#undef RT_S3
    if (!launched) return fail(RT_E_UNSUPPORTED, "conv (split fp16): window %dx%d stride %d not instantiated", sc.KH, sc.KW, sc.S);
    RT_LAUNCH_CHECK("conv_s3_kernel");
    return 0;
}

int enqueue_f16dw(const Launch& L, const SubConv& sc, rt::ConvArgs& a, bool& taken) {
    const rtConvPlan* plan = L.plan;
    if (!(plan->c3d_dw && plan->opt.dw != 0 && sc.KH == 3 && sc.KW == 3 && sc.S == 1 && sc.x_il8 && sc.y_il8 && !sc.zs_dev && sc.y_xstride == 1 &&
          (!plan->has_resid || sc.r_il8) && (plan->act == RT_ACT_NONE || plan->act == RT_ACT_ELU) && !sc.shift_dev))
        return 0;
    using Dw = rt::ConvF16DwCfg;
    const int dw_tiles_x = (int)rt::cdiv(sc.Wo, Dw::TX), dw_nkb = (int)rt::cdiv(sc.Cout, 32);
    const int64_t npairs = rt::cdiv(dw_tiles_x * (int)rt::cdiv(sc.Ho, Dw::TY), 2);
    int nseg = plan->opt.dw_nseg;
    double best = 1e30, fill = 1.0;
    for (int ns = 1; ns <= sc.nz; ns++) {
        const int seg = (int)rt::cdiv(sc.nz, ns);
        if (ns > 1 && seg < 4) break;
        if ((int)rt::cdiv(sc.nz, seg) != ns || (plan->opt.dw_nseg > 0 && ns != std::min(plan->opt.dw_nseg, sc.nz))) continue;
        const int64_t wgs = npairs * ns * dw_nkb * L.batch, rounds = rt::cdiv(wgs, (int64_t)device_cus());
        const double steps = seg + (ns > 1 ? 3.0 : 1.7), cost = (double)rounds * steps;
        if (cost < best - 1e-9) { best = cost; nseg = ns; fill = (double)wgs / (double)(rounds * device_cus()) * seg / steps; }
    }
    if (plan->opt.dw < 0 && fill < 0.6) return 0;
    taken = true;
    nseg = std::max(1, std::min(nseg, sc.nz));
    a.tiles_x = dw_tiles_x;
    a.dw_ntiles = a.tiles_x * (int)rt::cdiv(sc.Ho, Dw::TY);
    a.dw_cpc = plan->c3d_C / 16;
    a.nb_inner = dw_nkb;
    a.dw_seg = (int)rt::cdiv(sc.nz, nseg);
    a.dw_nseg = (int)rt::cdiv(sc.nz, a.dw_seg);
    const int64_t gx = npairs * a.dw_nseg * a.nb_inner;
    RT_REQUIRE(gx < (1ll << 31) && L.batch <= 65535, "rt_conv_enqueue: grid limit exceeded");
    dim3 gd((unsigned)gx, 1u, (unsigned)L.batch);
    const bool resident = a.dw_cpc <= 2, elu = plan->act == RT_ACT_ELU;
    if (plan->opt.trace)
        fprintf(stderr, "[rt] conv_f16dw<%d,%d,%d> grid %u x %u segments %d x %d slices, %d chunks per slice\n", resident ? 1 : 0,
                plan->has_resid ? 1 : 0, elu ? 1 : 0, gd.x, gd.z, a.dw_nseg, a.dw_seg, a.dw_cpc);
    with_bools([&](auto res, auto hr, auto el) { hipLaunchKernelGGL((rt::conv_f16dw_kernel<res, hr, el>), gd, dim3(512), 0, S(L.s), a); },
               resident, plan->has_resid, elu);
    RT_LAUNCH_CHECK("conv_f16dw_kernel");
    return 0;
}

int enqueue_f16mma(const Launch& L, const SubConv& sc, rt::ConvArgs& a, const ConvGrid& g) {
    const rtConvPlan* plan = L.plan;
    bool taken = false;
    if (int rc = enqueue_f16dw(L, sc, a, taken)) return rc;
    if (taken) return 0;
    if (sc.KH == 3 && sc.KW == 3 && sc.S == 1 && sc.x_il8 && sc.y_il8 && !sc.zs_dev && sc.TY == 4 && sc.y_xstride == 1 &&
        (plan->opt.r4 > 0 || (plan->opt.r4 < 0 && plan->is_conv3d && sc.Ho >= 12))) {
        dim3 g4 = g.fold(dim3((unsigned)(a.tiles_x * (int)rt::cdiv(sc.Ho, rt::ConvF16R4Cfg::TY)), g.grid.y, g.grid.z));
        if (plan->opt.trace) fprintf(stderr, "[rt] conv_f16r4 grid %u x %u x %u\n", g4.x, g4.y, g4.z);
        hipLaunchKernelGGL(rt::conv_f16r4_kernel, g4, dim3(256), 0, S(L.s), a);
        RT_LAUNCH_CHECK("conv_f16r4_kernel");
        return 0;
    }
    if (plan->opt.trace)
        fprintf(stderr, "[rt] conv_f16mma %dx%d s%d rows %d il8 x%d y%d r%d grid %u x %u x %u\n", sc.KH, sc.KW, sc.S, sc.TY, sc.x_il8,
                sc.y_il8, sc.r_il8, g.grid.x, g.grid.y, g.grid.z);
    const dim3 grid = g.fold(g.grid);
    if (sc.KH == 3 && sc.KW == 3 && sc.S == 1 && sc.TY == 4) {
        with_bools([&](auto xi, auto yi) { hipLaunchKernelGGL((rt::conv_f16mma_kernel<3, 3, 1, xi, yi, 4>), grid, dim3(256), 0, S(L.s), a); },
                   sc.x_il8, sc.y_il8);
        RT_LAUNCH_CHECK("conv_f16mma_kernel<3,3,1>");
        return 0;
    }
    if (sc.KH == 3 && sc.KW == 3 && sc.S == 2 && sc.TY == 4 && (sc.x_il8 || sc.y_il8)) {
        if (sc.x_il8 && sc.y_il8) hipLaunchKernelGGL((rt::conv_f16mma_kernel<3, 3, 2, true, true>), grid, dim3(256), 0, S(L.s), a);
// ... 345 lines not shown
```

Before: 2813.

## Store activations pre-split as fp16 hi/lo pairs across plain split convs

Extends the pre-split activation storage, previously limited to tensors between fused residual-tower blocks, to ordinary split-fp16 convolutions (3x3 s1/s2, 2x2). The s3 conv kernel gains template flags to read pre-split inputs directly into shared memory, read a pre-split residual, and write outputs as hi/lo fp16 pairs. This is meant to remove the per-load fp32-to-hi/lo conversion in consumers. In exchange, stored tensors double in size for those activations, and the engine pass gains more complex eligibility checks.

```diff
diff --git a/include/rt_stereo.h b/include/rt_stereo.h
--- a/include/rt_stereo.h
+++ b/include/rt_stereo.h
@@ -173,6 +173,8 @@
 
 int rt_resblock_plan_supports_split(const rtConvPlan* plan);
 int rt_resblock_plan_set_split(rtConvPlan* plan, int x_split, int y_split);
+int rt_conv_plan_supports_split(const rtConvPlan* plan);
+int rt_conv_plan_set_split(rtConvPlan* plan, int x_split, int y_split, int r_split);
 
 int rt_conv_plan_set_pitch(rtConvPlan* plan, int in_pitch, int out_pitch);
 int rt_conv_plan_set_batch_strides(rtConvPlan* plan, int64_t x_bstride, int64_t y_bstride, int64_t r_bstride);
diff --git a/redtail_amd/capi.py b/redtail_amd/capi.py
--- a/redtail_amd/capi.py
+++ b/redtail_amd/capi.py
@@ -168,6 +168,8 @@
     "rt_conv_enqueue_twin_input": (c_int, [c_void_p, c_void_p, c_void_p, c_void_p, c_int, c_void_p, c_int]),
     "rt_resblock_plan_supports_split": (c_int, [c_void_p]),
     "rt_resblock_plan_set_split": (c_int, [c_void_p, c_int, c_int]),
+    "rt_conv_plan_supports_split": (c_int, [c_void_p]),
+    "rt_conv_plan_set_split": (c_int, [c_void_p, c_int, c_int, c_int]),
     "rt_conv_enqueue": (c_int, [c_void_p, c_void_p, c_void_p, c_void_p, c_int, c_void_p]),
     "rt_conv_enqueue_hint": (c_int, [c_void_p, c_void_p, c_void_p, c_void_p, c_int, c_void_p, c_int]),
     "rt_conv_plan_workspace_bytes": (ctypes.c_size_t, [c_void_p, c_int]),
@@ -208,6 +210,9 @@
     return a
 
 
+_NEWEST_SYMBOLS = ("rt_conv_plan_supports_split", "rt_conv_plan_set_split")
+
+
 class KernelLib:
 
     def __init__(self, path=None):
@@ -219,6 +224,8 @@
         self.path = path
         self.lib = ctypes.CDLL(path, mode=ctypes.RTLD_GLOBAL)
         for name, (res, args) in KERNEL_SYMBOLS.items():
+            if name in _NEWEST_SYMBOLS and os.environ.get("RT_LIB_DIR") and not hasattr(self.lib, name):
+                continue
             fn = getattr(self.lib, name)
             fn.restype, fn.argtypes = res, args
         if not emulated and self.lib.rt_device_count() < 1:
@@ -485,6 +492,12 @@
 
     def set_split(self, x_split, y_split):
         self.klib.check(self.klib.lib.rt_resblock_plan_set_split(self.handle, int(x_split), int(y_split)), "rt_resblock_plan_set_split")
+
+    def split_caps(self):
+        return int(self.klib.lib.rt_conv_plan_supports_split(self.handle))
+
+    def set_conv_split(self, x_split, y_split, r_split=False):
+        self.klib.check(self.klib.lib.rt_conv_plan_set_split(self.handle, int(x_split), int(y_split), int(r_split)), "rt_conv_plan_set_split")
 
     def set_softarg(self, mode):
         self.klib.check(self.klib.lib.rt_conv_plan_set_softarg(self.handle, int(mode)), "rt_conv_plan_set_softarg")
diff --git a/redtail_amd/csrc/host/engine.cpp b/redtail_amd/csrc/host/engine.cpp
--- a/redtail_amd/csrc/host/engine.cpp
+++ b/redtail_amd/csrc/host/engine.cpp
@@ -457,6 +457,7 @@
     void assignInterleaved3D();
     void fuseSoftargmax3D();
     void fuseResBlocks();
+    void storePreSplit();
     void mergeSiamese();
     bool ok_ = false;
     bool half2_ = false;
@@ -510,6 +511,7 @@
     if (ok_) assignHalf3D();
     if (ok_) assignInterleaved3D();
     if (ok_) fuseSoftargmax3D();
+    if (ok_) storePreSplit();
     if (ok_) mergeSiamese();
     if (ok_) applySampleStrides();
     if (ok_) assignStreams();
@@ -1057,37 +1059,55 @@
     if (fused)
         log_.log(ILogger::Severity::kINFO, ("engine: " + std::to_string(fused) + " residual blocks fused into one launch each; " +
                                             std::to_string(ops_.size()) + " launches").c_str());
-    if (!fused || knob("RT_NO_RBD")) return;
-    auto tower = [&](const Op& op) { return op.kind == OpKind::kConv && op.plan && rt_resblock_plan_supports_split(op.plan) != 0; };
+}
+
+void EngineImpl::storePreSplit() {
+    if (knob("RT_NO_RBD") || exact_fp32_) return;
+    const bool tail = !knob("RT_NO_TAIL_SPLIT");
+    auto conv = [&](const Op& op) { return op.kind == OpKind::kConv && op.plan != nullptr; };
+    auto tower = [&](const Op& op) { return conv(op) && rt_resblock_plan_supports_split(op.plan) != 0; };
+    auto caps = [&](const Op& op) { return (tail && conv(op)) ? rt_conv_plan_supports_split(op.plan) : 0; };
     int nsplit = 0;
     for (size_t ia = 0; ia < ops_.size(); ia++) {
         const Op& a = ops_[ia];
-        if (!tower(a) || root(a.out) != a.out) continue;
+        if (!conv(a) || a.out < 0 || root(a.out) != a.out) continue;
         TensorImpl& t = *tensors_[a.out];
-        if (t.is_output || t.is_input || t.bstride != 0 || t.cpad != 0 || !t.il8 || t.f16) continue;
+        if (t.is_output || t.is_input || t.bstride != 0 || t.cpad != 0 || !t.il8 || t.f16 || t.split || t.dims.nbDims < 3 || t.dims.d[0] % 8 != 0) continue;
+        bool ok = true;
+        for (const auto& u : tensors_)
+            if (u->id != t.id && root(u->id) == t.id && (u->alias_off != 0 || u->bstride != 0)) ok = false;
         int readers = 0;
-        bool ok = true;
-        for (size_t j = 0; j < ops_.size(); j++) {
+        for (size_t j = 0; j < ops_.size() && ok; j++) {
             const Op& b = ops_[j];
-            bool reads = b.resid >= 0 && root(b.resid) == t.id;
-            for (int x : b.in) reads = reads || root(x) == t.id;
-            if (!reads) continue;
+            if (b.out >= 0 && root(b.out) == t.id) ok = ok && conv(b) && (tower(b) || (caps(b) & 2));
+            const bool as_r = b.resid >= 0 && root(b.resid) == t.id;
+            bool as_x = false;
+            for (int x : b.in) as_x = as_x || root(x) == t.id;
+            if (b.twin) {
+                for (int x : b.twin_in) as_x = as_x || root(x) == t.id;
+                if (b.twin_out >= 0 && root(b.twin_out) == t.id) ok = false;
+            }
+            if (!as_r && !as_x) continue;
             readers++;
-            ok = ok && j > ia && tower(b) && b.in.size() == 1 && root(b.in[0]) == t.id && b.resid >= 0 && root(b.resid) == t.id;
-        }
-        if (readers == 1 && ok) { t.split = true; nsplit++; }
+            if (!conv(b) || j <= ia || b.in.size() != 1) { ok = false; break; }
+            if (tower(b)) ok = ok && as_x && as_r;
+            else ok = ok && !tower(a) && (!as_x || (caps(b) & 1)) && (!as_r || (caps(b) & 4));
+        }
+        if (ok && readers > 0) { t.split = true; nsplit++; }
     }
     if (!nsplit) return;
     for (Op& op : ops_) {
-        if (!tower(op)) continue;
-        const bool xs = tensors_[root(op.in[0])]->split, ys = tensors_[root(op.out)]->split;
-        if ((xs || ys) && rt_resblock_plan_set_split(op.plan, xs, ys) != 0) {
+        if (!conv(op)) continue;
+        const bool xs = tensors_[root(op.in[0])]->split, ys = tensors_[root(op.out)]->split, rs = op.resid >= 0 && tensors_[root(op.resid)]->split;
+        if (!xs && !ys && !rs) continue;
+        const int rc = tower(op) ? rt_resblock_plan_set_split(op.plan, xs, ys) : rt_conv_plan_set_split(op.plan, xs, ys, rs);
+        if (rc != 0) {
             log_.log(ILogger::Severity::kERROR, rt_last_error_string());
             ok_ = false;
             return;
         }
     }
-    log_.log(ILogger::Severity::kINFO, ("engine: " + std::to_string(nsplit) + " tensors between tower blocks stored pre-split (fp16 hi / lo operand pairs)").c_str());
+    log_.log(ILogger::Severity::kINFO, ("engine: " + std::to_string(nsplit) + " activation tensors stored pre-split (fp16 hi / lo operand pairs)").c_str());
 }
 
 void EngineImpl::mergeSiamese() {
diff --git a/redtail_amd/csrc/kernels/conv_mfma.hip.h b/redtail_amd/csrc/kernels/conv_mfma.hip.h
--- a/redtail_amd/csrc/kernels/conv_mfma.hip.h
+++ b/redtail_amd/csrc/kernels/conv_mfma.hip.h
@@ -56,6 +56,7 @@
     int dw_seg, dw_nseg, dw_cpc, dw_ntiles;
     const float* x2;
     int x2_from;
+    int r_split;
 };
 
 #define RT_WG_TILE_NB(p, tile, zi, n, nblk)                                                         \
diff --git a/redtail_amd/csrc/kernels/conv_split.hip.h b/redtail_amd/csrc/kernels/conv_split.hip.h
--- a/redtail_amd/csrc/kernels/conv_split.hip.h
+++ b/redtail_amd/csrc/kernels/conv_split.hip.h
@@ -258,10 +258,12 @@
 #ifndef RT_S3_WAVES
 #define RT_S3_WAVES(S) ((S) == 2 ? 2 : 4)
 #endif
-template <int KH, int KW, int S, bool XIL, bool YIL, int NW = 4, typename TIN = float, typename TOUT = float>
+template <int KH, int KW, int S, bool XIL, bool YIL, int NW = 4, typename TIN = float, typename TOUT = float, bool XSP = false, bool YSP = false>
 __global__ void __launch_bounds__(64 * NW * (S3Cfg<KH, KW, S, NW>::KS_MAX)) RT_WAVES_PER_EU(RT_S3_WAVES(S)) conv_s3_kernel(ConvArgs p) {
     using Cfg = S3Cfg<KH, KW, S, NW>;
     constexpr bool XF16 = std::is_same<TIN, _Float16>::value, YF16 = std::is_same<TOUT, _Float16>::value;
+    static_assert(!XSP || (XIL && !XF16 && NW == 4), "pre-split input: interleaved fp32-sized tensors, 4 waves");
+    static_assert(!YSP || (YIL && !YF16), "pre-split output: interleaved fp32-sized tensors");
     constexpr unsigned ESX = Io<TIN>::ES, ESY = Io<TOUT>::ES;
     static_assert(!XIL || !XF16, "interleaved fp16 input: conv_f16mma_kernel");
     constexpr int TY = Cfg::TY, TX = Cfg::TX, CC = Cfg::CC, TAPS = Cfg::TAPS, PC = Cfg::PC, PCL = Cfg::PCL, PXB = Cfg::PXB;
@@ -310,7 +312,7 @@
     const int act = p.act;
 
     const int sg = wv & 3, spart = wv >> 2;
-    const int* __restrict__ tab = p.ch_off + (int64_t)ch_row * p.CinPad + 4 * sg;
+    const int* __restrict__ tab = p.ch_off + (int64_t)ch_row * p.CinPad + (XSP ? 8 * (sg >> 1) : 4 * sg);
     unsigned voff[NKP];
     int lidx[NKP], xcol[NKP];
     const int* __restrict__ shtab = p.ch_shift ? p.ch_shift + (int64_t)ch_row * p.CinPad + 4 * sg : nullptr;
@@ -321,9 +323,10 @@
         const int iy = ty0 * S - pad_y + pr, ix = tx0 * S - pad_x + pc;
         const bool own = pidx < Cfg::NPIX && lane + 64 * k < NKP * 64;
         xcol[k] = ix;
-        voff[k] = (own && iy >= 0 && iy < p.Hi && ix >= 0 && ix < p.Wi) ? (unsigned)(iy * p.x_pitch + ix) * (XIL ? 16u : ESX) : kBufOOB;
+        if constexpr (XSP) voff[k] = (own && iy >= 0 && iy < p.Hi && ix >= 0 && ix < p.Wi) ? (unsigned)(iy * p.x_pitch + ix) * 32u + 16u * (sg & 1) : kBufOOB;
+        else voff[k] = (own && iy >= 0 && iy < p.Hi && ix >= 0 && ix < p.Wi) ? (unsigned)(iy * p.x_pitch + ix) * (XIL ? 16u : ESX) : kBufOOB;
         const int col = S == 2 ? (pc & 1) * Cfg::PCH + (pc >> 1) : pc;
-        lidx[k] = own ? (pr * PCL + col) * PXB + sg * 8 : -1;
+        lidx[k] = own ? (pr * PCL + col) * PXB + (XSP ? 32 * (sg & 1) + 16 * (sg >> 1) : sg * 8) : -1;
     }
     const char* __restrict__ wsrc = reinterpret_cast<const char*>(p.w) + (w_off + ((int64_t)nblk * nchunks) * Cfg::W_SLOTS) * 16;
     const buf_rsrc rs_w = make_buf(wsrc);
@@ -331,7 +334,12 @@
     f32x4 rin[NKP];
     f32x4 rw[NK_W];
     auto prefetch = [&](int ch) {
-        if constexpr (XIL) {
+        if constexpr (XSP) {
+            const int off = tab[ch * CC];
+            const buf_rsrc rs = make_buf(xb, off >= 0);
+#pragma unroll
+            for (int k = 0; k < NKP; k++) rin[k] = buf_load4(rs, voff[k], (unsigned)off * 4u);
+        } else if constexpr (XIL) {
             const int off = tab[ch * CC];
             const int sh = shtab ? shtab[ch * CC] : 0;
             const buf_rsrc rs = make_buf(xb, off >= 0);
@@ -364,7 +372,9 @@
 #pragma unroll
         for (int k = 0; k < NKP; k++) {
             if (lidx[k] < 0) continue;
-            if constexpr (XF16) {
+            if constexpr (XSP) {
+                *reinterpret_cast<f32x4*>(sIn + lidx[k]) = rin[k];
+            } else if constexpr (XF16) {
                 f16x4 h;
 #pragma unroll
                 for (int j = 0; j < 4; j++) h[j] = (_Float16)rin[k][j];
@@ -392,7 +402,18 @@
     f32x4 rr[4];
     if (p.resid != nullptr && kgi == 0) {
         const buf_rsrc rs_r = make_buf(elem_ptr(p.resid, r_il ? (int64_t)n * p.r_bstride + (YF16 ? r_off_il8 : r_off_il4) : rbase, ESY));
-        if (r_il && YF16) {
+        if (!YF16 && p.r_split) {
+            const buf_rsrc rs_s = make_buf(elem_ptr(p.resid, (int64_t)n * p.r_bstride + 2 * r_off_il4, ESY));
+            const unsigned vo = inb ? (unsigned)(oy * p.y_ystride + ox * p.y_xstride) * 32u + 8u * kg : kBufOOB;
+#pragma unroll
+            for (int q = 0; q < 4; q++) {
+                const unsigned so = (unsigned)((cb + 8 * q) * rs32) * 4u;
+                const unsigned vq = (cb + 8 * q + 4 * kg < p.Cout) ? vo : kBufOOB;
+                const f16x4 h = __builtin_bit_cast(f16x4, buf_load2(rs_s, vq, so)), l = __builtin_bit_cast(f16x4, buf_load2(rs_s, vq, so + 16u));
+#pragma unroll
+                for (int e = 0; e < 4; e++) rr[q][e] = fmaf((float)l[e], kSplitInv, (float)h[e]);
+            }
+        } else if (r_il && YF16) {
             const unsigned vo = inb ? (unsigned)((oy * p.y_ystride + ox * p.y_xstride) * 8 + 4 * kg) * 2u : kBufOOB;
 #pragma unroll
             for (int q = 0; q < 4; q++) {
@@ -478,7 +499,7 @@
             }
     }
 
-    const buf_rsrc rs_y = make_buf(elem_ptr(p.y, (YIL && !YF16) ? (int64_t)n * p.y_bstride + y_off_il4 : ybase, ESY));
+    const buf_rsrc rs_y = make_buf(elem_ptr(p.y, (YIL && !YF16) ? (int64_t)n * p.y_bstride + (YSP ? 2 : 1) * y_off_il4 : ybase, ESY));
     auto epilogue = [&](auto ACT) {
 #pragma unroll
         for (int q = 0; q < 4; q++) {
@@ -487,7 +508,12 @@
 #pragma unroll
             for (int e = 0; e < 4; e++)
                 o[e] = apply_act_fast(acc_m[4 * q + e] + (bv[e] + rr[q][e]), decltype(ACT)::value);
-            if constexpr (YIL && YF16) {
+            if constexpr (YSP) {
+                const S3Split sp = s3_split(o);
+                const unsigned vs = (inb && cb + 8 * q + 4 * kg < p.Cout) ? (unsigned)(oy * p.y_ystride + ox * p.y_xstride) * 32u + 8u * kg : kBufOOB;
+                buf_store2(__builtin_bit_cast(f32x2_t, sp.hi), rs_y, vs, (unsigned)((cb + 8 * q) * cs32) * 4u);
+                buf_store2(__builtin_bit_cast(f32x2_t, sp.lo), rs_y, vs, (unsigned)((cb + 8 * q) * cs32) * 4u + 16u);
+            } else if constexpr (YIL && YF16) {
                 const unsigned vo = (inb && cb + 8 * q + 4 * kg < p.Cout) ? (unsigned)((oy * p.y_ystride + ox * p.y_xstride) * 8 + 4 * kg) * 2u : kBufOOB;
                 u32x2_t w2;
 #pragma unroll
diff --git a/redtail_amd/csrc/rt_capi.hip b/redtail_amd/csrc/rt_capi.hip
--- a/redtail_amd/csrc/rt_capi.hip
+++ b/redtail_amd/csrc/rt_capi.hip
@@ -1310,6 +1310,7 @@
     float* rbd_w1_dev = nullptr;
     float* rbd_w2_dev = nullptr;
     int x_split = 0, y_split = 0;
+    int r_split = 0;
     float* rbh_w1_dev = nullptr;
     float* rbh_w2_dev = nullptr;
     int w_f16 = 0;
@@ -1621,24 +1622,27 @@
 }
 
 template <typename T> constexpr const char* type_tag() { return sizeof(T) == 2 ? "f16" : "f32"; }
-template <int KH, int KW, int S, bool XIL, bool YIL, int NW = 4, typename TIN = float, typename TOUT = float>
+template <int KH, int KW, int S, bool XIL, bool YIL, int NW = 4, typename TIN = float, typename TOUT = float, bool XSP = false, bool YSP = false>
 void launch_s3(dim3 grid, int ks, int64_t per_cu, hipStream_t st, const rt::ConvArgs& a, int trace = 0) {
     using Cfg = rt::S3Cfg<KH, KW, S, NW>;
     ks = Cfg::max_groups(ks);
     while (ks > 1 && std::min<int64_t>(per_cu, 4) * ks * Cfg::GRP_BYTES > 160 * 1024) ks = Cfg::max_groups(ks - 1);
-    if (trace)
-        fprintf(stderr, "[rt] conv_s3<%d,%d,%d,%d,%d,%d,%s,%s> r%d grid %u x %u x %u ks %d\n", KH, KW, S, (int)XIL, (int)YIL, NW, type_tag<TIN>(),
-                type_tag<TOUT>(), a.r_il8, grid.x, grid.y, grid.z, ks);
+    if (trace) {
+        char sp[32] = "";
+        if (trace >= 2) std::snprintf(sp, sizeof sp, " split x%d y%d r%d", (int)XSP, (int)YSP, a.r_split);
+        fprintf(stderr, "[rt] conv_s3<%d,%d,%d,%d,%d,%d,%s,%s> r%d grid %u x %u x %u ks %d%s\n", KH, KW, S, (int)XIL, (int)YIL, NW, type_tag<TIN>(),
+                type_tag<TOUT>(), a.r_il8, grid.x, grid.y, grid.z, ks, sp);
+    }
 #ifndef HIPEMU
     static std::atomic<unsigned long long> done{0};
     int dev = 0;
     if (hipGetDevice(&dev) == hipSuccess && dev >= 0 && dev < 64 && !((done.load(std::memory_order_acquire) >> dev) & 1ull)) {
-        (void)hipFuncSetAttribute(reinterpret_cast<const void*>(&rt::conv_s3_kernel<KH, KW, S, XIL, YIL, NW, TIN, TOUT>),
+        (void)hipFuncSetAttribute(reinterpret_cast<const void*>(&rt::conv_s3_kernel<KH, KW, S, XIL, YIL, NW, TIN, TOUT, XSP, YSP>),
                                   hipFuncAttributeMaxDynamicSharedMemorySize, Cfg::KS_MAX * Cfg::GRP_BYTES);
         done.fetch_or(1ull << dev, std::memory_order_release);
     }
 #endif
-    hipLaunchKernelGGL((rt::conv_s3_kernel<KH, KW, S, XIL, YIL, NW, TIN, TOUT>), grid, dim3(64 * NW * ks), (size_t)ks * Cfg::GRP_BYTES, st, a);
+    hipLaunchKernelGGL((rt::conv_s3_kernel<KH, KW, S, XIL, YIL, NW, TIN, TOUT, XSP, YSP>), grid, dim3(64 * NW * ks), (size_t)ks * Cfg::GRP_BYTES, st, a);
 }
 
 int device_cus() {
@@ -1900,6 +1904,27 @@
     const SubConv& sc = plan->subs[0];
     return sc.rb && sc.x_il8 && sc.y_il8 && !sc.x_f16 && !sc.y_f16 && plan->cin == 32 && plan->rb_cmid == 32 && sc.Cout == 32 && plan->rb_act1 == 1 &&
            plan->act == 1 && !(plan->flags & RT_CONV_EXACT_FP32);
+}
+
+static int s3_split_caps(const rtConvPlan* plan) {
+    if (!plan || plan->subs.size() != 1 || !plan->is2d || (plan->flags & RT_CONV_EXACT_FP32) || env_int("RT_NO_RBD", 0) != 0) return 0;
+    const SubConv& sc = plan->subs[0];
+    if (!sc.split3 || sc.rb || sc.direct || sc.dp4 || sc.x_f16 || sc.y_f16 || !sc.x_il8 || sc.TY != 4 || sc.NW != 4 || sc.shift_dev || sc.nz < 1) return 0;
+    if (!((sc.KH == 3 && sc.KW == 3 && (sc.S == 1 || sc.S == 2)) || (sc.KH == 2 && sc.KW == 2 && sc.S == 1))) return 0;
+    return (plan->cin % 8 == 0 ? 1 : 0) | ((sc.y_il8 && sc.Cout % 8 == 0) ? 2 : 0) | ((plan->has_resid && sc.r_il8 && sc.Cout % 8 == 0) ? 4 : 0);
+}
+extern "C" int rt_conv_plan_supports_split(const rtConvPlan* plan) { return s3_split_caps(plan); }
+extern "C" int rt_conv_plan_set_split(rtConvPlan* plan, int x_split, int y_split, int r_split) {
+    RT_REQUIRE(plan, "rt_conv_plan_set_split: null plan");
+    RT_REQUIRE(!plan->rb_w1_dev, "rt_conv_plan_set_split: a residual block takes rt_resblock_plan_set_split");
+    if (!x_split && !y_split && !r_split) { plan->x_split = plan->y_split = plan->r_split = 0; return 0; }
+    const int caps = s3_split_caps(plan);
+    if ((x_split && !(caps & 1)) || (y_split && !(caps & 2)) || (r_split && !(caps & 4)))
+        return fail(RT_E_UNSUPPORTED, "rt_conv_plan_set_split: no kernel reads / writes a pre-split %s tensor for this plan (caps %d: interleaved 2-D plans of "
+                    "fp32 tensors, 3x3 stride 1 / 2 and transposed 3x3 stride 2, channels in groups of 8, no folded cost volume)",
+                    x_split && !(caps & 1) ? "input" : (y_split && !(caps & 2) ? "output" : "residual"), caps);
+    plan->x_split = x_split != 0; plan->y_split = y_split != 0; plan->r_split = r_split != 0;
+    return 0;
 }
 
 extern "C" int rt_deconv2d_plan_create(rtConvPlan** out, const rtConv2dDesc* d, const void* weights, const void* bias) {
@@ -2833,11 +2858,11 @@
     RT_REQUIRE(plan, "rt_conv_plan_set_layouts: null plan");
     ExactScope exact_scope(plan->flags);
     struct KeepOnFailure {
-        rtConvPlan* p; int softarg, xs, ys; bool ok = false;
-        ~KeepOnFailure() { if (!ok) { p->softarg = softarg; p->x_split = xs; p->y_split = ys; } }
-    } keep{plan, plan->softarg, plan->x_split, plan->y_split};
+        rtConvPlan* p; int softarg, xs, ys, rsp; bool ok = false;
+        ~KeepOnFailure() { if (!ok) { p->softarg = softarg; p->x_split = xs; p->y_split = ys; p->r_split = rsp; } }
+    } keep{plan, plan->softarg, plan->x_split, plan->y_split, plan->r_split};
     plan->softarg = 0;
-    plan->x_split = plan->y_split = 0;
+    plan->x_split = plan->y_split = plan->r_split = 0;
     if (!x_il8 && !y_il8 && !r_il8) {
         if (plan->is_conv3d && plan->subs.size() == 1 && plan->subs[0].f16mma)
             if (int rc = switch_conv3d_f16mma(plan, false)) return rc;
@@ -3133,6 +3158,7 @@
     a.r_cstride = sc.r_cstride ? sc.r_cstride : sc.y_cstride;
     a.r_bstride = plan->r_bstride ? plan->r_bstride : plan->y_bstride;
     a.r_il8 = sc.r_il8;
+    a.r_split = plan->r_split;
     a.batch = L.batch; a.cin_real = sc.cin_real; a.x_cstride = (int64_t)sc.Hi * a.x_pitch;
     return a;
 }
@@ -3354,6 +3380,22 @@
         RT_S3H(3, 3, 1) RT_S3H(3, 3, 2) RT_S3H(1, 1, 1) RT_S3H(1, 2, 1) RT_S3H(2, 1, 1) RT_S3H(2, 2, 1)
 #undef RT_S3H
     }
+    if (plan->x_split || plan->y_split) {
+        RT_REQUIRE(s3_split_caps(plan) != 0, "rt_conv_enqueue: pre-split tensors on a plan that has no kernel for them");
+#define RT_S3SP(kh, kw, st)                                                                                                                          \
+    if (!launched && sc.KH == kh && sc.KW == kw && sc.S == st) {                                                                                     \
+        if (plan->x_split && plan->y_split) launch_s3<kh, kw, st, true, true, 4, float, float, true, true>(grid, ks, per_cu, S(L.s), a, trace);      \
+        else if (plan->x_split && sc.y_il8) launch_s3<kh, kw, st, true, true, 4, float, float, true, false>(grid, ks, per_cu, S(L.s), a, trace);     \
+        else if (plan->x_split) launch_s3<kh, kw, st, true, false, 4, float, float, true, false>(grid, ks, per_cu, S(L.s), a, trace);                \
+        else launch_s3<kh, kw, st, true, true, 4, float, float, false, true>(grid, ks, per_cu, S(L.s), a, trace);                                    \
+        launched = true;                                                                                                                             \
+    }
+        RT_S3SP(3, 3, 1) RT_S3SP(3, 3, 2) RT_S3SP(2, 2, 1)
+#undef RT_S3SP
+        RT_REQUIRE(launched, "rt_conv_enqueue: pre-split form of this window not instantiated");
+        RT_LAUNCH_CHECK("conv_s3_kernel (pre-split)");
+        return 0;
+    }
 #ifdef RT_EXPERIMENTAL
     if (!launched && sc.KH == 3 && sc.KW == 3 && sc.S == 1 && sc.TY == 8) {
         with_bools([&](auto xi, auto yi) { launch_s3<3, 3, 1, xi, yi, 8>(grid, ks, per_cu, S(L.s), a, trace); }, sc.x_il8, sc.y_il8);
```

After: 2818, median of 2. About the same (+0.2%).
